# jacobkrantz/IVLN-CE

Hardware: AMD Instinct MI355X
Metric: env-steps/sec (batched MapCMA fwd+bwd) at 1/2/4/8 MI355X; t-nDTW parity (higher is better)
Workload: dtype f32

## Files before the change

### include/ivln_hip.h

```cpp
#ifndef IVLN_HIP_H
#define IVLN_HIP_H
#include <stdint.h>
#ifdef __cplusplus
extern "C" {
#endif

#define IVLN_OK 0
#define IVLN_E_INVALID -1
#define IVLN_E_HIP -2
#define IVLN_E_KEYSPACE -3
#define IVLN_E_CAPACITY -4
#define IVLN_E_UNSUPPORTED -5

const char* ivln_strerror(int code);
int ivln_version(void);

typedef struct ivln_mapper ivln_mapper;

int ivln_mapper_create(int B_max, int H, int W, double vfov_rad, double height_m, double width_m,
                       double res_m, int64_t world_capacity, int64_t table_cells, ivln_mapper** out);
int ivln_mapper_destroy(ivln_mapper* m);
int ivln_mapper_reset(ivln_mapper* m, void* stream);

int ivln_mapper_set_launch_width(ivln_mapper* m, int local_blocks, int world_blocks);

int ivln_mapper_frames(const float* pose, const double* orientation, int B, float* T, float* rot,
                       void* stream);

int ivln_mapper_step(ivln_mapper* m, const float* depth, const uint8_t* labels, const float* T,
                     const float* pose, const float* rot, const uint8_t* not_done, int B,
                     uint8_t* occ_out, uint8_t* sem_out, void* stream);

int ivln_mapper_step_posed(ivln_mapper* m, const float* depth, const uint8_t* labels, const float* pose,
                           const double* orientation, const uint8_t* not_done, int B, uint8_t* occ_out,
                           uint8_t* sem_out, float* T_out, float* rot_out, void* stream);

int ivln_mapper_step_begin(ivln_mapper* m, const float* depth, const float* pose, const double* orientation,
                           const uint8_t* not_done, int B, uint8_t* occ_out, float* T_out, float* rot_out, void* stream);
int ivln_mapper_step_finish(ivln_mapper* m, const float* depth, const uint8_t* labels, const float* T, const float* pose,
                            const float* rot, const uint8_t* not_done, int B, uint8_t* occ_out, uint8_t* sem_out, void* stream);

int ivln_mapper_known_begin(ivln_mapper* m, const uint8_t* not_done, int B, void* stream);
int ivln_mapper_load_known(ivln_mapper* m, int b, const float* xyz, const uint8_t* sem, int64_t n,
                           void* stream);
int ivln_mapper_known_raster(ivln_mapper* m, const float* pose, const float* rot, int B,
                             uint8_t* occ_out, uint8_t* sem_out, void* stream);

int ivln_mapper_status(ivln_mapper* m, int64_t* world_n, void* stream);
int ivln_mapper_world_export(ivln_mapper* m, float* xyz, uint32_t* meta, int64_t* rank,
                             int64_t max_n, int64_t* n_out, void* stream);


enum { IVLN_A_MK = 0,
       IVLN_A_KM = 1,
       IVLN_A_NCHW_P = 2    };
enum { IVLN_B_CONV = 0,
       IVLN_B_CONV1X1 = 1,
       IVLN_B_KN = 2,
       IVLN_B_NK = 3,
       IVLN_B_IM2COL_T = 4,
       IVLN_B_CONVT = 5,
       IVLN_B_CONV_K3 = 6,
       IVLN_B_CONV_K7 = 7,
       IVLN_B_CONV_K2 = 8   };
enum { IVLN_D_NCHW = 0,
       IVLN_D_DENSE = 1,
       IVLN_D_NCHW_UP2 = 2,
       IVLN_D_NCHW_UP2X4 = 3  };

typedef struct ivln_gemm_desc {
    const float* A;
    const float* B;
    float* D;
    int M, N, K;
    int amode, bmode, dmode;
    int64_t lda, ldb;
    int Cin, Hin, Win, Hout, Wout, stride, pad, dil;
    const int32_t* koff;
    const int32_t* kpos;
    int HoWo;
    int Ctot;
    int64_t in_img_stride;
    int64_t sDm, sDn;
    const float* scale;
    const float* shift;
    const float* residual;
    int relu, accumulate;
    int splits;
    float* ws;
    int64_t ws_floats;
    int defer_epilogue;
    int* splits_used;
    int tile_override;
    const float* A_packed;
    int no_xcd_remap;
    int grp_imgs;
    int64_t a_grp_stride, a_packed_grp_stride;
    int no_wide_epilogue;
    float* stat_partials;
    int* stat_tiles;
    const void* A_split;
    int64_t a_split_grp_stride;
    int split_ok;
    const int32_t* img_run_flags;
    const void* fuse_A_split;
    int64_t fuse_a_grp_stride;
    const float* fuse_scale;
    const float* fuse_shift;
    int fuse_M;
    int residual_after_relu;
    int real_taps;
} ivln_gemm_desc;

int ivln_gemm_f32(const ivln_gemm_desc* desc, void* stream);
int64_t ivln_conv_split_words(int M, int Cin, int KS);
int ivln_conv_split_weights_f32(const float* W, int M, int Cin, int KS, void* out, void* stream);
int64_t ivln_conv_stem_split_words(int M, int Cin);
int ivln_conv_stem_split_weights_f32(const float* W, int M, int Cin, void* out, void* stream);
int ivln_conv_split_counters(double* flops, long long* launches, int reset);
int ivln_conv_split_kinds(long long* out4, int reset);

int ivln_family_timing_begin(int max_launches);
int ivln_family_timing_end(double* total_ms, int* launches, int* dropped);
int ivln_family_timing_report(char* buf, int cap);
const char* ivln_family_kernel_names(void);
int64_t ivln_conv_packed_floats(int M, int Cin, int KS);
int ivln_conv_pack_weights_f32(const float* W, int M, int Cin, int KS, float* out, void* stream);

typedef struct ivln_gn_conv_desc {
    const float* x;
    int splits;
    int64_t slab_stride;
    const float* gamma;
    const float* beta;
    const float* x2;
    int splits2;
    int64_t slab_stride2;
    const float* gamma2;
    const float* beta2;
    const float* residual;
    int N, C, H, W, groups;
    float eps;
    int relu;
    int pool;
    float* act_out;
    const float* wa;
    int Cout_a, ka, stride_a, pad_a;
    float* ya;
    const float* wb;
    int Cout_b, stride_b;
    float* yb;
    const float* x0;
    int splits0;
    int64_t slab_stride0;
    int C0, groups0;
    const float* gamma0;
    const float* beta0;
    const float* w0;
} ivln_gn_conv_desc;
int ivln_gn_conv_f32(const ivln_gn_conv_desc* d, void* stream);

typedef struct ivln_depthnet_op {
    int kind;
    int Cin, Cout, ks, stride, pad;
    int Hin, Win;
    int wout_shift;
    int M;
    int WCT, WPT, P, KW;
    int kwg;
    int n_ctg, n_ptg;
    int ksteps;
    int cs, wp;
    int src_off, nslab, slab_stride;
    int st_off, st_parts;
    int gamma_off, beta_off;
    int src2_off, st2_off, st2_parts, gamma2_off, beta2_off;
    int res_off;
    int relu, pool, avg_in;
    int act_out_off;
    int dst_off, dst_slab_stride;
    int st_out_off, st_out_parts;
    int w_off;
    int barrier_before;
} ivln_depthnet_op;
int ivln_depth_net_f32(const ivln_depthnet_op* ops_dev, const ivln_depthnet_op* ops_host, int n_ops, const float* weights,
                       const float* params, const float* depth, int64_t depth_img_stride, float* arena, int64_t arena_stride,
                       float* out, int64_t out_img_stride, int N, float eps, void* sync_ws, void* stream);
int ivln_depth_net_status(const void* sync_ws, void* stream);
int ivln_depth_net_reset(void* sync_ws, void* stream);
int ivln_host_device_ptr(void* host, void** dev);

typedef struct ivln_nconv_desc {
    const float* x;
    const float* stats;
    int parts;
    const float* gamma;
    const float* beta;
    const float* x2;
    const float* stats2;
    int parts2;
    const float* gamma2;
    const float* beta2;
    const float* residual;
    int N, C, H, W, groups;
    float eps;
    int relu;
    float* act_out;
    const float* wa;
    int Cout_a, ka, groups_a;
    float* ya;
    float* stats_a;
    const float* wb;
    int Cout_b, groups_b;
    float* yb;
    float* stats_b;
    int rows_per_block;
    int stride_a, stride_b;
} ivln_nconv_desc;
int ivln_nconv_f32(const ivln_nconv_desc* d, void* stream);

int ivln_groupnorm_f32(const float* x, const float* gamma, const float* beta, const float* residual,
// ... 210 lines not shown
```

### ivln-ce_amd/csrc/conv_bf3.hip

```cpp
#include <stdlib.h>

#include <type_traits>

#include "gemm_common.h"
#include "residency.h"

namespace {

typedef __bf16 bf16x8 __attribute__((ext_vector_type(8)));
typedef int v4i __attribute__((ext_vector_type(4)));
typedef int v2i __attribute__((ext_vector_type(2)));

constexpr int PIXB = 112;
constexpr int CB = 16;

__host__ __device__ constexpr int bf3_taps_padded(int KS) { return KS == 7 ? 54 : (KS == 3 ? 9 : (KS == 2 ? 4 : 1)); }
__host__ __device__ constexpr int bf3_gx0(int KS) { return KS == 2 ? 0 : 4; }
__host__ __device__ constexpr int bf3_xoff(int KS) { return KS == 2 ? 0 : 4 - KS / 2; }
__host__ __device__ constexpr int bf3_stage_chunks(int KS) { return KS == 1 ? 4 : 1; }

__device__ __forceinline__ uint32_t bf16_rne_bits(float v, bool& fin) {
    const uint32_t u = __float_as_uint(v);
    fin = (u & 0x7F800000u) != 0x7F800000u;
    uint32_t hb = (u + 0x7FFFu + ((u >> 16) & 1u)) & 0xFFFF0000u;
// ... 720 lines not shown
                for (int pl = 0; pl < 3; ++pl) abuf[slot][pl] = load_a(s0 + r + DA, pl);
                if (r == (KK > 4 ? 1 : 0)) load_patch(min(c + 1, c1 - 1));
                __builtin_amdgcn_sched_barrier(0);
            }
        }
    }
#ifdef BF3_TIMING
    const unsigned long long ts2 = lane == 0 ? wall_clock64() : 0ull;
#endif
    __syncthreads();
    float* const red = reinterpret_cast<float*>(smem);
#pragma unroll
    for (int tn = 0; tn < TN; ++tn)
#pragma unroll
        for (int r = 0; r < 16; ++r)
            red[(wave * 32 + (r & 3) + 8 * (r >> 2) + 4 * half) * LDT + tn * 32 + l31] = acc[tn][r];
    __syncthreads();
    if constexpr (UP) {
        if (t < 16 * 16 * TN) {
            const int r = t / (16 * TN), j = t % (16 * TN);
            const int ml = 2 * r, nl = 2 * j;
            const int ph = nl / PTW, pw = nl % PTW;
            const int ho = ho0 + ph, wo = wo0 + pw;
            float4 v = make_float4(0.f, 0.f, 0.f, 0.f);
#pragma unroll
            for (int w = 0; w < NW; ++w) {
                const float2 u0 = *reinterpret_cast<const float2*>(red + (w * 32 + ml) * LDT + nl);
                const float2 u1 = *reinterpret_cast<const float2*>(red + (w * 32 + ml + 1) * LDT + nl);
                v.x += u0.x, v.y += u1.x, v.z += u0.y, v.w += u1.y;
            }
            if (m0 + ml < p.M && img0 < nimg && ho < p.Hout && wo < p.Wout) {
                const int co = (m0 + ml) >> 2, a = r & 1;
                const int64_t addr = (((int64_t)img0 * p.Ctot + co) * (2 * p.Hout) + 2 * ho + a) * (2 * p.Wout) + 2 * wo;
                if (p.scale) {
                    const float sc = p.scale[co], sh = p.shift[co];
                    v.x = fmaf(v.x, sc, sh), v.y = fmaf(v.y, sc, sh), v.z = fmaf(v.z, sc, sh), v.w = fmaf(v.w, sc, sh);
                } else if (p.shift) {
                    const float sh = p.shift[co];
                    v.x += sh, v.y += sh, v.z += sh, v.w += sh;
                }
                if (p.residual) {
                    const float4 rr = *reinterpret_cast<const float4*>(p.residual + addr);
                    v.x += rr.x, v.y += rr.y, v.z += rr.z, v.w += rr.w;
                }
                if (p.accumulate) {
                    const float4 rr = *reinterpret_cast<const float4*>(p.D + addr);
                    v.x += rr.x, v.y += rr.y, v.z += rr.z, v.w += rr.w;
                }
                if (p.relu) v.x = fmaxf(v.x, 0.f), v.y = fmaxf(v.y, 0.f), v.z = fmaxf(v.z, 0.f), v.w = fmaxf(v.w, 0.f);
                *reinterpret_cast<float4*>(p.D + addr) = v;
            }
        }
    } else if (t < 32 * 8 * TN) {
        const int ml = t / (8 * TN), c4 = t % (8 * TN);
        const int m = m0 + ml, nl = 4 * c4;
        const int ph = nl / PTW, pw = nl % PTW;
        const int ho = ho0 + ph, wo = wo0 + pw;
        float4 v = make_float4(0.f, 0.f, 0.f, 0.f);
#pragma unroll
        for (int w = 0; w < NW; ++w) {
            const float4 u = *reinterpret_cast<const float4*>(red + (w * 32 + ml) * LDT + nl);
            v.x += u.x, v.y += u.y, v.z += u.z, v.w += u.w;
        }
        if (m < p.M && img0 < nimg && ho < p.Hout && wo < p.Wout) {
            const int64_t addr = ((int64_t)img0 * p.Ctot + m) * p.HoWo + ho * p.Wout + wo;
            const int me = p.grp_imgs > 0 ? (img0 / p.grp_imgs) * p.M + m : m;
            if (p.scale) {
                const float sc = p.scale[me], sh = p.shift[me];
                v.x = fmaf(v.x, sc, sh), v.y = fmaf(v.y, sc, sh), v.z = fmaf(v.z, sc, sh), v.w = fmaf(v.w, sc, sh);
            } else if (p.shift) {
                const float sh = p.shift[me];
                v.x += sh, v.y += sh, v.z += sh, v.w += sh;
            }
            if (p.residual) {
                const float4 rr = *reinterpret_cast<const float4*>(p.residual + addr);
                v.x += rr.x, v.y += rr.y, v.z += rr.z, v.w += rr.w;
            }
            if (p.accumulate) {
                const float4 rr = *reinterpret_cast<const float4*>(p.D + addr);
                v.x += rr.x, v.y += rr.y, v.z += rr.z, v.w += rr.w;
            }
            if (p.relu) v.x = fmaxf(v.x, 0.f), v.y = fmaxf(v.y, 0.f), v.z = fmaxf(v.z, 0.f), v.w = fmaxf(v.w, 0.f);
            *reinterpret_cast<float4*>(p.D + addr) = v;
        }
    }
#ifdef BF3_TIMING
    if (lane == 0) {
        __builtin_amdgcn_s_waitcnt(0);
        const unsigned long long ts3 = wall_clock64();
        const int b = ((blockIdx.y * gridDim.x + blockIdx.x) * NW + wave) & 8191;
        g_bf3_stamp[b * 8 + 0] = ts1 - ts0;
        g_bf3_stamp[b * 8 + 1] = ts2 - ts1;
        g_bf3_stamp[b * 8 + 2] = ts3 - ts2;
        g_bf3_stamp[b * 8 + 3] = ts0;
        g_bf3_stamp[b * 8 + 4] = t_stage;
    }
#endif
}

template <int PTH, int PTW, int TN = 2, int KS = 3>
int launch_bf3_ks_tile(const ivln_gemm_desc& d, hipStream_t s, const unsigned char* a_split, int64_t grp_bytes, int nimg) {
    constexpr int NPIX = (PTH + KS - 1) * (PTW + KS - 1), WREG = (NPIX * PIXB + 15) & ~15, RED = 8 * 32 * (32 * TN + 4) * 4;
    constexpr size_t lds = (size_t)(8 * WREG > RED ? 8 * WREG : RED);
    static_assert(lds <= 160 * 1024, "patch regions do not fit");
    auto kern = k_conv_bf3_ks<PTH, PTW, TN, KS>;
    static bool attr_done = false;
    if (!attr_done) {
        if (hipFuncSetAttribute((const void*)kern, hipFuncAttributeMaxDynamicSharedMemorySize, (int)lds) != hipSuccess) return IVLN_E_HIP;
        attr_done = true;
    }
    const int tiles_w = d.Wout / PTW, tiles_h = d.Hout / PTH;
    dim3 grid(tiles_w * tiles_h * nimg, (d.M + 31) / 32, 1);
    IVLN_LAUNCH_FAMILY_NAMED("k_conv_bf3_ks", kern, grid, dim3(512), lds, s, d, a_split, (long long)grp_bytes, tiles_w, tiles_h, nimg);
    return IVLN_OK;
}

int bf3_ks_launch(ivln_gemm_desc& d, hipStream_t s, int nimg, int mode, int tn_pin = 0) {
    if (d.Cin % CB != 0 || d.Cin < 8 * CB || d.stat_partials || d.splits > 1) return IVLN_E_UNSUPPORTED;
    if (d.bmode == BMODE_CONV_K2) {
        if (d.grp_imgs > 0 || (d.Wout != 8 && d.Wout != 16 && d.Wout != 32) || d.Hout % (64 / d.Wout) != 0 || (d.in_img_stride & 3) ||
            (((uintptr_t)d.B) & 15) || (int64_t)nimg * d.in_img_stride * 4 >= (int64_t)1 << 31)
            return IVLN_E_UNSUPPORTED;
        const int64_t wgs2 = (int64_t)(d.N / 64) * ((d.M + 31) / 32);
        if (mode == 0 && (wgs2 > 2 * (int64_t)ivln_cu_count() || wgs2 < ivln_cu_count() / 4)) return IVLN_E_UNSUPPORTED;
        d.splits = 1;
        const unsigned char* a2 = (const unsigned char*)d.A_split;
        const int64_t gb2 = d.a_split_grp_stride * 4;
        if (d.Wout == 8) return launch_bf3_ks_tile<8, 8, 2, 2>(d, s, a2, gb2, nimg);
        if (d.Wout == 16) return launch_bf3_ks_tile<4, 16, 2, 2>(d, s, a2, gb2, nimg);
        return launch_bf3_ks_tile<2, 32, 2, 2>(d, s, a2, gb2, nimg);
    }
    if (d.Wout != 8 && d.Wout != 16 && d.Wout != 32) return IVLN_E_UNSUPPORTED;
    const int64_t wgs = (int64_t)(d.N / 64) * ((d.M + 31) / 32);
    constexpr int tn_env = 0;
    const bool small = tn_pin ? tn_pin == 1 : (tn_env ? tn_env == 1 : 2 * wgs <= ivln_cu_count());
    const int pth = (small ? 32 : 64) / d.Wout;
    if (d.Hout % pth != 0 || (d.in_img_stride & 3) || (((uintptr_t)d.B) & 15)) return IVLN_E_UNSUPPORTED;
    if ((int64_t)nimg * d.in_img_stride * 4 >= (int64_t)1 << 31) return IVLN_E_UNSUPPORTED;
    if (d.grp_imgs > 0 && nimg % d.grp_imgs != 0) return IVLN_E_UNSUPPORTED;
    if (mode == 0 && (wgs > 2 * (int64_t)ivln_cu_count() || wgs < ivln_cu_count() / 4)) return IVLN_E_UNSUPPORTED;
    const int64_t gb = d.a_split_grp_stride * 4;
    d.splits = 1;
    const unsigned char* a = (const unsigned char*)d.A_split;
    if (small) {
        if (d.Wout == 8) return launch_bf3_ks_tile<4, 8, 1>(d, s, a, gb, nimg);
        if (d.Wout == 16) return launch_bf3_ks_tile<2, 16, 1>(d, s, a, gb, nimg);
        return launch_bf3_ks_tile<1, 32, 1>(d, s, a, gb, nimg);
    }
    if (d.Wout == 8) return launch_bf3_ks_tile<8, 8>(d, s, a, gb, nimg);
    if (d.Wout == 16) return launch_bf3_ks_tile<4, 16>(d, s, a, gb, nimg);
    return launch_bf3_ks_tile<2, 32>(d, s, a, gb, nimg);
}

template <bool WT>
__global__ __launch_bounds__(WT ? 256 : 512, 2) void k_conv1x1_bf3_ks(const ivln_gemm_desc p, const unsigned char* a_split, long long a_grp_bytes) {
    constexpr int NW = WT ? 4 : 8, TN = 4, DA = 4, BN = 128;
    constexpr int LDT = BN + 4;
    constexpr unsigned OOB = 0x80000000u;
    extern __shared__ __attribute__((aligned(16))) unsigned char smem[];
    const int t = threadIdx.x, lane = t & 63;
    const int wave = __builtin_amdgcn_readfirstlane(t >> 6);
    const int half = lane >> 5, l31 = lane & 31;
    const BlockId bid = xcd_block_id(p.no_xcd_remap);
    const int n0 = WT ? (bid.y * NW + wave) * BN : bid.y * BN, m0 = bid.x * 32;
    const int nch = p.Cin / CB;
    const int HW = p.HoWo;
    const int cpw = WT ? nch : (nch + NW - 1) / NW;
    const int c0 = WT ? 0 : min(nch, wave * cpw), c1 = WT ? nch : min(nch, c0 + cpw);
    const int n_img0 = min(n0, p.N - 1) / HW;
    const int grp = p.grp_imgs > 0 ? n_img0 / p.grp_imgs : 0;

    const int nq = n0 + 4 * l31;
    const int qimg = nq / HW, qpp = nq - qimg * HW;
    const unsigned hw4 = (unsigned)HW * 4u;
    const unsigned xvo = nq < p.N ? (unsigned)(((int64_t)qimg * p.in_img_stride + qpp + (int64_t)(8 * half) * HW) * 4) : OOB;
    const __amdgpu_buffer_rsrc_t rB = bf3_rsrc(p.B);
    auto load_x = [&](int c, v4i (&xb)[8]) {
        const int so = c * CB * HW * 4;
#pragma unroll
        for (int j = 0; j < 8; ++j) xb[j] = __builtin_amdgcn_raw_buffer_load_b128(rB, (int)xvo, so + j * (int)hw4, 0);
    };
    const int mt = min(m0 / 32, (p.M + 31) / 32 - 1);
    const __amdgpu_buffer_rsrc_t rA = bf3_rsrc(a_split + (int64_t)grp * a_grp_bytes + (int64_t)mt * nch * (3 * 1024));
    const int c_last = max(c1 - 1, 0);
    auto load_a = [&](int c, v4i (&ab)[3]) {
#pragma unroll
        for (int pl = 0; pl < 3; ++pl) ab[pl] = __builtin_amdgcn_raw_buffer_load_b128(rA, (min(c, c_last) * 3 + pl) * 1024 + lane * 16, 0, 0);
    };
    f32x16 acc[TN];
#pragma unroll
    for (int tn = 0; tn < TN; ++tn)
#pragma unroll
        for (int i = 0; i < 16; ++i) acc[tn][i] = 0.f;

#ifdef BF3_TIMING
    const unsigned long long ts0 = lane == 0 ? wall_clock64() : 0ull;
    unsigned long long ts1 = ts0, tc_split = 0, tc_load = 0, tc_mfma = 0;
#endif
    if (c0 < c1 && (!WT || n0 < p.N)) {
        v4i xb[2][8], ab[DA][3];
#pragma unroll
        for (int d = 0; d < DA; ++d) load_a(c0 + d, ab[d]);
        load_x(c0, xb[0]);
        load_x(min(c0 + 1, c_last), xb[1]);
#ifdef BF3_TIMING
        __builtin_amdgcn_s_waitcnt(0);
        ts1 = lane == 0 ? wall_clock64() : 0ull;
#endif
        for (int cc = c0; cc < c1; cc += DA) {
#pragma unroll
            for (int k = 0; k < DA; ++k) {
                const int c = cc + k;
                v4i bq[TN][3];
                bf16x8 a[3];
#ifdef BF3_TIMING
                const unsigned long long tl0 = __builtin_readcyclecounter();
#endif
                if (c < c1) {
#pragma unroll
                    for (int e = 0; e < 4; ++e)
#pragma unroll
                        for (int i = 0; i < 4; ++i) {
                            uint32_t H, M, L;
#ifdef BF3_PROBE_NO_SPLIT
                            H = xb[k & 1][2 * i][e], M = xb[k & 1][2 * i + 1][e], L = H ^ M;
#else
                            split3_pair(__int_as_float(xb[k & 1][2 * i][e]), __int_as_float(xb[k & 1][2 * i + 1][e]), H, M, L);
#endif
                            bq[e][0][i] = (int)H, bq[e][1][i] = (int)M, bq[e][2][i] = (int)L;
                        }
#pragma unroll
                    for (int pl = 0; pl < 3; ++pl) a[pl] = __builtin_bit_cast(bf16x8, ab[k][pl]);
                }
                __builtin_amdgcn_sched_barrier(0);
#ifdef BF3_TIMING
                const unsigned long long tl1 = __builtin_readcyclecounter();
                __builtin_amdgcn_sched_barrier(0);
#endif
                load_x(min(c + 2, c_last), xb[k & 1]);
                load_a(c + DA, ab[k]);
                __builtin_amdgcn_sched_barrier(0);
#ifdef BF3_TIMING
                const unsigned long long tl2 = __builtin_readcyclecounter();
                __builtin_amdgcn_sched_barrier(0);
#endif
                if (c < c1) {
#define IVLN_BF3_PROD(PA, PB)                            \
    _Pragma("unroll") for (int tn = 0; tn < TN; ++tn)    \
        acc[tn] = __builtin_amdgcn_mfma_f32_32x32x16_bf16(a[PA], __builtin_bit_cast(bf16x8, bq[tn][PB]), acc[tn], 0, 0, 0)
#ifdef BF3_PROBE_NO_MFMA
                    IVLN_BF3_PROD(0, 0);
#else
                    IVLN_BF3_PROD(0, 2);
                    IVLN_BF3_PROD(1, 1);
                    IVLN_BF3_PROD(2, 0);
                    IVLN_BF3_PROD(0, 1);
                    IVLN_BF3_PROD(1, 0);
                    IVLN_BF3_PROD(0, 0);
#endif
#undef IVLN_BF3_PROD
                }
#ifdef BF3_TIMING
                __builtin_amdgcn_sched_barrier(0);
                const unsigned long long tl3 = __builtin_readcyclecounter();
                tc_split += tl1 - tl0, tc_load += tl2 - tl1, tc_mfma += tl3 - tl2;
#endif
            }
        }
    }
#ifdef BF3_TIMING
    const unsigned long long ts2 = lane == 0 ? wall_clock64() : 0ull;
#endif
    const bool up = p.dmode == DMODE_NCHW_UP2X4;
    if (WT && up) {
        const int n = n0 + 4 * l31;
        if (n < p.N) {
            const int img = n / HW, pp = n - img * HW;
            const int ho = pp / p.Wout, wo = pp - ho * p.Wout;
#pragma unroll
            for (int r = 0; r < 16; r += 2) {
                const int m = m0 + 4 * half + (r & 3) + 8 * (r >> 2);
                if (m >= p.M) continue;
                const int co = m >> 2, a = (m >> 1) & 1;
                const int64_t addr = (((int64_t)img * p.Ctot + co) * (2 * p.Hout) + 2 * ho + a) * (2 * p.Wout) + 2 * wo;
                float v[8];
#pragma unroll
                for (int e = 0; e < 4; ++e) v[2 * e] = acc[e][r], v[2 * e + 1] = acc[e][r + 1];
                const float sc = p.scale ? p.scale[co] : 1.f, sh = p.shift ? p.shift[co] : 0.f;
#pragma unroll
                for (int e = 0; e < 8; ++e) v[e] = p.scale ? fmaf(v[e], sc, sh) : v[e] + sh;
                if (p.residual) {
                    const float4 r0 = *reinterpret_cast<const float4*>(p.residual + addr), r1 = *reinterpret_cast<const float4*>(p.residual + addr + 4);
                    v[0] += r0.x, v[1] += r0.y, v[2] += r0.z, v[3] += r0.w, v[4] += r1.x, v[5] += r1.y, v[6] += r1.z, v[7] += r1.w;
                }
                if (p.relu) {
#pragma unroll
                    for (int e = 0; e < 8; ++e) v[e] = fmaxf(v[e], 0.f);
                }
                *reinterpret_cast<float4*>(p.D + addr) = make_float4(v[0], v[1], v[2], v[3]);
                *reinterpret_cast<float4*>(p.D + addr + 4) = make_float4(v[4], v[5], v[6], v[7]);
            }
        }
    } else
    if constexpr (WT) {
        const int n = n0 + 4 * l31;
        const int img = min(n, p.N - 1) / HW, pp = n - img * HW;
        const int mrem = n < p.N ? p.M - m0 - 4 * half : 0;
        const int me0 = (p.grp_imgs > 0 ? (img / p.grp_imgs) * p.M : 0) + m0 + 4 * half;
        const unsigned off0 = (unsigned)(((img * p.Ctot + m0 + 4 * half) * HW + pp) * 4);
        const __amdgpu_buffer_rsrc_t rR = bf3_rsrc(p.residual), rS = bf3_rsrc(p.scale), rH = bf3_rsrc(p.shift), rD = bf3_rsrc(p.D);
        const bool has_res = p.residual != nullptr, has_sc = p.scale != nullptr, has_sh = p.shift != nullptr;
        const float relu_lo = p.relu ? 0.f : -__builtin_huge_valf();
        const bool res_post = p.residual_after_relu != 0;
        v4i rres[16];
        float esc[16], esh[16];
#pragma unroll
        for (int r = 0; r < 16; ++r) {
            const int cs = (r & 3) + 8 * (r >> 2);
            const bool ok = cs < mrem;
            esc[r] = __int_as_float(__builtin_amdgcn_raw_buffer_load_b32(rS, ok && has_sc ? me0 * 4 : (int)OOB, cs * 4, 0));
            esh[r] = __int_as_float(__builtin_amdgcn_raw_buffer_load_b32(rH, ok && has_sh ? me0 * 4 : (int)OOB, cs * 4, 0));
            rres[r] = __builtin_amdgcn_raw_buffer_load_b128(rR, ok && has_res ? (int)off0 : (int)OOB, cs * HW * 4, 0);
        }
#pragma unroll
        for (int r = 0; r < 16; ++r) {
            const int cs = (r & 3) + 8 * (r >> 2);
            float4 v = make_float4(acc[0][r], acc[1][r], acc[2][r], acc[3][r]);
            const float sc = has_sc ? esc[r] : 1.f, sh = esh[r];
            v.x = fmaf(v.x, sc, sh), v.y = fmaf(v.y, sc, sh), v.z = fmaf(v.z, sc, sh), v.w = fmaf(v.w, sc, sh);
            const float r0 = __int_as_float(rres[r][0]), r1 = __int_as_float(rres[r][1]), r2 = __int_as_float(rres[r][2]), r3 = __int_as_float(rres[r][3]);
            v.x += res_post ? 0.f : r0, v.y += res_post ? 0.f : r1, v.z += res_post ? 0.f : r2, v.w += res_post ? 0.f : r3;
            const float lo = relu_lo;
            v.x = fmaxf(v.x, lo), v.y = fmaxf(v.y, lo), v.z = fmaxf(v.z, lo), v.w = fmaxf(v.w, lo);
            v.x += res_post ? r0 : 0.f, v.y += res_post ? r1 : 0.f, v.z += res_post ? r2 : 0.f, v.w += res_post ? r3 : 0.f;
            v4i o;
            o[0] = __float_as_int(v.x), o[1] = __float_as_int(v.y), o[2] = __float_as_int(v.z), o[3] = __float_as_int(v.w);
            __builtin_amdgcn_raw_buffer_store_b128(o, rD, cs < mrem ? (int)off0 : (int)OOB, cs * HW * 4, 0);
            BF3_STORE_GUARD();
        }
    } else if (up) {
        float* const red = reinterpret_cast<float*>(smem);
#pragma unroll
        for (int tn = 0; tn < TN; ++tn)
#pragma unroll
            for (int r = 0; r < 16; ++r)
                red[(wave * 32 + (r & 3) + 8 * (r >> 2) + 4 * half) * LDT + tn * 32 + l31] = acc[tn][r];
        __syncthreads();
#pragma unroll
        for (int it = 0; it < 2; ++it) {
            const int item = t + it * 512, r = item >> 6, j = item & 63;
            const int ml = 2 * r, nl = 2 * j, n = n0 + nl;
            const int e0 = nl & 3, q = nl >> 2;
            float4 v = make_float4(0.f, 0.f, 0.f, 0.f);
#pragma unroll
            for (int w = 0; w < NW; ++w) {
                const float* r0 = red + (w * 32 + ml) * LDT + q;
                const float* r1 = r0 + LDT;
                v.x += r0[e0 * 32], v.y += r1[e0 * 32], v.z += r0[(e0 + 1) * 32], v.w += r1[(e0 + 1) * 32];
            }
            if (m0 + ml < p.M && n < p.N) {
                const int img = n / HW, pp = n - img * HW;
                const int ho = pp / p.Wout, wo = pp - ho * p.Wout;
                const int co = (m0 + ml) >> 2, a = r & 1;
                const int64_t addr = (((int64_t)img * p.Ctot + co) * (2 * p.Hout) + 2 * ho + a) * (2 * p.Wout) + 2 * wo;
                if (p.scale) {
                    const float sc = p.scale[co], sh = p.shift[co];
                    v.x = fmaf(v.x, sc, sh), v.y = fmaf(v.y, sc, sh), v.z = fmaf(v.z, sc, sh), v.w = fmaf(v.w, sc, sh);
                } else if (p.shift) {
                    const float sh = p.shift[co];
                    v.x += sh, v.y += sh, v.z += sh, v.w += sh;
                }
                if (p.residual) {
                    const float4 rr = *reinterpret_cast<const float4*>(p.residual + addr);
                    v.x += rr.x, v.y += rr.y, v.z += rr.z, v.w += rr.w;
                }
                if (p.relu) v.x = fmaxf(v.x, 0.f), v.y = fmaxf(v.y, 0.f), v.z = fmaxf(v.z, 0.f), v.w = fmaxf(v.w, 0.f);
                *reinterpret_cast<float4*>(p.D + addr) = v;
            }
        }
    } else {
    constexpr int ITEMS = 2;
    v4i rres[ITEMS];
    float esc[ITEMS], esh[ITEMS];
    int eoff[ITEMS];
    const __amdgpu_buffer_rsrc_t rR = bf3_rsrc(p.residual), rS = bf3_rsrc(p.scale), rH = bf3_rsrc(p.shift);
    const bool has_res = p.residual != nullptr, has_sc = p.scale != nullptr, has_sh = p.shift != nullptr;
    auto request = [&](int it) {
        const int item = t + it * 512, ml = item >> 5, q = item & 31;
        const int m = m0 + ml, n = n0 + 4 * q;
        const bool ok = m < p.M && n < p.N;
        const int img = n / HW, pp = n - img * HW;
        const int off = (img * p.Ctot + m) * HW + pp;
        const int me = p.grp_imgs > 0 ? (img / p.grp_imgs) * p.M + m : m;
        eoff[it] = ok ? off : -1;
        esc[it] = __int_as_float(__builtin_amdgcn_raw_buffer_load_b32(rS, ok && has_sc ? me * 4 : (int)OOB, 0, 0));
        esh[it] = __int_as_float(__builtin_amdgcn_raw_buffer_load_b32(rH, ok && has_sh ? me * 4 : (int)OOB, 0, 0));
        rres[it] = __builtin_amdgcn_raw_buffer_load_b128(rR, ok && has_res ? off * 4 : (int)OOB, 0, 0);
    };
#pragma unroll
    for (int it = 0; it < ITEMS; ++it) request(it);
    float* const red = reinterpret_cast<float*>(smem);
#pragma unroll
    for (int tn = 0; tn < TN; ++tn)
#pragma unroll
        for (int r = 0; r < 16; ++r)
            red[(wave * 32 + (r & 3) + 8 * (r >> 2) + 4 * half) * LDT + tn * 32 + l31] = acc[tn][r];
    __syncthreads();
#pragma unroll
    for (int it = 0; it < ITEMS; ++it) {
        const int item = t + it * 512, ml = item >> 5, q = item & 31;
        float4 v = make_float4(0.f, 0.f, 0.f, 0.f);
#pragma unroll
        for (int w = 0; w < NW; ++w) {
            const float* rr = red + (w * 32 + ml) * LDT + q;
            v.x += rr[0], v.y += rr[32], v.z += rr[64], v.w += rr[96];
        }
        if (eoff[it] >= 0) {
            const int64_t addr = eoff[it];
            const float sc = esc[it], sh = esh[it];
            if (p.scale) v.x = fmaf(v.x, sc, sh), v.y = fmaf(v.y, sc, sh), v.z = fmaf(v.z, sc, sh), v.w = fmaf(v.w, sc, sh);
            else if (p.shift) v.x += sh, v.y += sh, v.z += sh, v.w += sh;
            const bool res_pre = p.residual && !p.residual_after_relu, res_post = p.residual && p.residual_after_relu;
            if (res_pre)
                v.x += __int_as_float(rres[it][0]), v.y += __int_as_float(rres[it][1]), v.z += __int_as_float(rres[it][2]),
                    v.w += __int_as_float(rres[it][3]);
            if (p.accumulate) {
                const float4 ra = *reinterpret_cast<const float4*>(p.D + addr);
                v.x += ra.x, v.y += ra.y, v.z += ra.z, v.w += ra.w;
            }
            if (p.relu) v.x = fmaxf(v.x, 0.f), v.y = fmaxf(v.y, 0.f), v.z = fmaxf(v.z, 0.f), v.w = fmaxf(v.w, 0.f);
            if (res_post)
                v.x += __int_as_float(rres[it][0]), v.y += __int_as_float(rres[it][1]), v.z += __int_as_float(rres[it][2]),
                    v.w += __int_as_float(rres[it][3]);
            *reinterpret_cast<float4*>(p.D + addr) = v;
        }
    }
    }
#ifdef BF3_TIMING
    if (lane == 0) {
        __builtin_amdgcn_s_waitcnt(0);
        const unsigned long long ts3 = wall_clock64();
        const int b = ((blockIdx.y * gridDim.x + blockIdx.x) * NW + wave) & 8191;
        g_bf3_stamp[b * 8 + 0] = ts1 - ts0;
        g_bf3_stamp[b * 8 + 1] = ts2 - ts1;
        g_bf3_stamp[b * 8 + 2] = ts3 - ts2;
        g_bf3_stamp[b * 8 + 3] = ts0;
        g_bf3_stamp[b * 8 + 4] = tc_split;
        g_bf3_stamp[b * 8 + 5] = tc_load;
        g_bf3_stamp[b * 8 + 6] = tc_mfma;
    }
#endif
}

int bf3_1x1_ks_launch(ivln_gemm_desc& d, hipStream_t s, int mode, int form_pin = -1) {
    if (d.stride != 1 || d.pad != 0 || d.Cin % CB != 0 || d.Cin < 4 * CB || d.stat_partials || d.splits > 1) return IVLN_E_UNSUPPORTED;
    if ((d.HoWo & 3) || (d.in_img_stride & 3) || ((((uintptr_t)d.B) | ((uintptr_t)d.D) | ((uintptr_t)d.residual)) & 15)) return IVLN_E_UNSUPPORTED;
    const int64_t nimg = d.N / d.HoWo;
    if (nimg * d.in_img_stride * 4 >= (int64_t)1 << 31 || nimg * d.Ctot * d.HoWo * 4 >= (int64_t)1 << 31) return IVLN_E_UNSUPPORTED;
    if (d.grp_imgs > 0 && ((int64_t)d.grp_imgs * d.HoWo) % 128 != 0) return IVLN_E_UNSUPPORTED;
    const int nch = d.Cin / CB;
    constexpr const char* form_env = nullptr;
    bool wt = nch <= 16;
    constexpr int maxwg0 = 2;
    if (nch == 32 && (int64_t)((d.N + 127) / 128) * ((d.M + 31) / 32) > maxwg0 * (int64_t)ivln_cu_count()) wt = true;
    if (form_env) wt = form_env[0] == 'w';
    if (form_pin >= 0) wt = form_pin == 1;
    if (wt && nch > 64) wt = false;
    if (wt && d.accumulate) return IVLN_E_UNSUPPORTED;
    const int64_t mtiles = (d.M + 31) / 32;
    const int64_t wgs = wt ? (int64_t)((d.N + 511) / 512) * mtiles : (int64_t)((d.N + 127) / 128) * mtiles;
    constexpr int maxwg_env = 2;
    if ((d.N + 127) / 128 > 65535) return IVLN_E_UNSUPPORTED;
    if (mode == 0) {
        if (!wt && (d.Cin < 32 * CB || wgs > maxwg_env * (int64_t)ivln_cu_count() || wgs < ivln_cu_count() / 2)) return IVLN_E_UNSUPPORTED;
        if (wt && wgs < ivln_cu_count()) return IVLN_E_UNSUPPORTED;
    }
    d.splits = 1;
    const unsigned char* a = (const unsigned char*)d.A_split;
    const long long gb = (long long)(d.a_split_grp_stride * 4);
    if (wt) {
        constexpr size_t lds = 0;
        dim3 grid((unsigned)mtiles, (unsigned)((d.N + 511) / 512), 1);
        IVLN_LAUNCH_FAMILY(k_conv1x1_bf3_ks<true>, grid, dim3(256), lds, s, d, a, gb);
    } else {
        constexpr size_t lds = (size_t)8 * 32 * (128 + 4) * 4;
        static bool attr_done = false;
        if (!attr_done) {
            if (hipFuncSetAttribute((const void*)k_conv1x1_bf3_ks<false>, hipFuncAttributeMaxDynamicSharedMemorySize, (int)lds) != hipSuccess) return IVLN_E_HIP;
            attr_done = true;
        }
        dim3 grid((unsigned)mtiles, (unsigned)((d.N + 127) / 128), 1);
        IVLN_LAUNCH_FAMILY(k_conv1x1_bf3_ks<false>, grid, dim3(512), lds, s, d, a, gb);
    }
    return IVLN_OK;
}

__global__ __launch_bounds__(256) void k_conv_bf3_pack(const float* __restrict__ W, int M, int Cin, int KS, uint16_t* __restrict__ out,
                                                       int64_t total) {
    const int64_t idx = (int64_t)blockIdx.x * 256 + threadIdx.x;
    if (idx >= total) return;
    const int KK = KS * KS, KKP = bf3_taps_padded(KS), nch = (Cin + CB - 1) / CB;
    const int e = (int)(idx & 7), lane = (int)((idx >> 3) & 63);
    int64_t q = idx >> 9;
    const int pl = (int)(q % 3);
    q /= 3;
    const int r = (int)(q % KKP);
    q /= KKP;
    const int c = (int)(q % nch);
    const int mt = (int)(q / nch);
    const int m = mt * 32 + (lane & 31), ci = c * CB + (lane >> 5) * 8 + e;
    const float v = (m < M && ci < Cin && r < KK) ? W[((int64_t)m * Cin + ci) * KK + r] : 0.f;
    uint32_t h, mm, l;
    split3(v, h, mm, l);
    out[idx] = (uint16_t)(pl == 0 ? h : (pl == 1 ? mm : l));
}

template <int KS, int TM, int WM, int WN, int PTH, int PTW, int IMGS, int DA, int ST = 1>
int launch_bf3(const ivln_gemm_desc& d, hipStream_t s, const unsigned char* a_split, int64_t grp_bytes, int nimg, int cps) {
    constexpr int NTB = 64 * WM * WN, BM = 32 * TM * WM, BN = 64 * WN;
    constexpr int PH = ST == 2 ? PTH + 1 : PTH + KS - 1, PWR = ST == 2 ? PTW + 1 : PTW + KS - 1;
    constexpr int NPIX = IMGS * (ST == 2 ? 4 : 1) * PH * PWR * bf3_stage_chunks(KS);
    constexpr size_t lds = (size_t)(NPIX * PIXB > 32 * (BN + 4) * 4 ? NPIX * PIXB : 32 * (BN + 4) * 4);
    if constexpr (lds > 160 * 1024) {
        return IVLN_E_UNSUPPORTED;
    } else {
    auto kern = k_conv_bf3<KS, TM, WM, WN, PTH, PTW, IMGS, DA, false, ST>;
    static bool attr_done = false;
    if (!attr_done) {
        if (hipFuncSetAttribute((const void*)kern, hipFuncAttributeMaxDynamicSharedMemorySize, (int)lds) != hipSuccess) return IVLN_E_HIP;
        attr_done = true;
    }
    const int tiles_w = (d.Wout + PTW - 1) / PTW, tiles_h = (d.Hout + PTH - 1) / PTH;
    const int groups = (nimg + IMGS - 1) / IMGS;
    dim3 grid(tiles_w * tiles_h * groups, (d.M + BM - 1) / BM, d.splits);
    IVLN_LAUNCH_FAMILY_NAMED("k_conv_bf3", kern, grid, dim3(NTB), lds, s, d, a_split, (long long)grp_bytes, tiles_w, tiles_h, nimg, cps);
    return IVLN_OK;
    }
}

template <int TM, int WM, int WN, int DA>
int launch_bf3_fused(const ivln_gemm_desc& d, hipStream_t s, const unsigned char* a_split, int64_t grp_bytes, int nimg) {
    constexpr int KS = 3, PTW = 32, NTB = 64 * WM * WN, BM = 32 * TM * WM, BN = 64 * WN, PTH = BN / PTW;
    static_assert(NTB == 256, "four waves");
    constexpr int NPIX = (PTH + 2) * (PTW + 2);
    constexpr size_t ybytes = (size_t)BM * (BN + 4) * 4, lds = (size_t)NPIX * PIXB > ybytes ? (size_t)NPIX * PIXB : ybytes;
    auto kern = k_conv_bf3<KS, TM, WM, WN, PTH, PTW, 1, DA, true>;
    static bool attr_done = false;
    if (!attr_done) {
        if (hipFuncSetAttribute((const void*)kern, hipFuncAttributeMaxDynamicSharedMemorySize, (int)lds) != hipSuccess) return IVLN_E_HIP;
        attr_done = true;
    }
    const int tiles_w = d.Wout / PTW, tiles_h = d.Hout / PTH;
    dim3 grid(tiles_w * tiles_h * nimg, 1, 1);
    const int nch = d.Cin / CB;
    IVLN_LAUNCH_FAMILY_NAMED("k_conv_bf3", kern, grid, dim3(NTB), lds, s, d, a_split, (long long)grp_bytes, tiles_w, tiles_h, nimg, nch);
    return IVLN_OK;
}

struct Bf3Px { int pth, ptw, imgs; };
inline Bf3Px bf3_px(int BN, int Wout) {
    const int ptw = Wout > 16 ? 32 : (Wout > 8 ? 16 : 8);
    const int pth = ptw == 32 ? BN / 32 : (ptw == 16 ? (BN >= 256 ? 16 : 8) : 8);
    return {pth, ptw, BN / (ptw * pth)};
}

template <int KS, int TM, int WM, int WN, int DA, int ST = 1>
int launch_bf3_px(const ivln_gemm_desc& d, hipStream_t s, const unsigned char* a, int64_t gb, int nimg, int cps) {
    constexpr int BN = 64 * WN;
    if constexpr (ST == 2) {
        static_assert(KS == 3 && (BN == 128 || BN == 256), "stride-2 tiles");
        if constexpr (BN == 256) {
            if (d.Wout > 16) return launch_bf3<KS, TM, WM, WN, 8, 32, 1, DA, 2>(d, s, a, gb, nimg, cps);
            if (d.Wout > 8) return launch_bf3<KS, TM, WM, WN, 16, 16, 1, DA, 2>(d, s, a, gb, nimg, cps);
            return launch_bf3<KS, TM, WM, WN, 8, 8, 4, DA, 2>(d, s, a, gb, nimg, cps);
        } else {
            if (d.Wout > 16) return launch_bf3<KS, TM, WM, WN, 4, 32, 1, DA, 2>(d, s, a, gb, nimg, cps);
            if (d.Wout > 8) return launch_bf3<KS, TM, WM, WN, 8, 16, 1, DA, 2>(d, s, a, gb, nimg, cps);
            return launch_bf3<KS, TM, WM, WN, 8, 8, 2, DA, 2>(d, s, a, gb, nimg, cps);
        }
    } else
    if constexpr (BN == 512 && KS == 1) {
        return IVLN_E_UNSUPPORTED;
    } else if constexpr (BN == 512) {
        if (d.Wout > 16) return launch_bf3<KS, TM, WM, WN, 16, 32, 1, DA>(d, s, a, gb, nimg, cps);
        if (d.Wout > 8) return launch_bf3<KS, TM, WM, WN, 16, 16, 2, DA>(d, s, a, gb, nimg, cps);
        if constexpr (KS == 3) return launch_bf3<KS, TM, WM, WN, 8, 8, 8, DA>(d, s, a, gb, nimg, cps);
        return IVLN_E_UNSUPPORTED;
    } else if constexpr (BN == 256) {
        if (d.Wout > 16) return launch_bf3<KS, TM, WM, WN, 8, 32, 1, DA>(d, s, a, gb, nimg, cps);
        if (d.Wout > 8) return launch_bf3<KS, TM, WM, WN, 16, 16, 1, DA>(d, s, a, gb, nimg, cps);
        return launch_bf3<KS, TM, WM, WN, 8, 8, 4, DA>(d, s, a, gb, nimg, cps);
    } else {
        if (d.Wout > 16) return launch_bf3<KS, TM, WM, WN, 4, 32, 1, DA>(d, s, a, gb, nimg, cps);
        if (d.Wout > 8) return launch_bf3<KS, TM, WM, WN, 8, 16, 1, DA>(d, s, a, gb, nimg, cps);
        return launch_bf3<KS, TM, WM, WN, 8, 8, 2, DA>(d, s, a, gb, nimg, cps);
    }
}

constexpr int kBf3Cfgs = 7;
constexpr int kBf3BM[kBf3Cfgs] = {32, 64, 64, 128, 64, 128, 32};
constexpr int kBf3BN[kBf3Cfgs] = {512, 512, 256, 256, 128, 128, 256};

template <int KS>
int launch_bf3_ks(const ivln_gemm_desc& d, hipStream_t s, const unsigned char* a, int64_t gb, int nimg, int cfg, int cps) {
    constexpr int DA2 = KS == 1 || KS == 2 ? 2 : 3, DA1 = KS == 1 || KS == 2 ? 4 : (KS == 7 ? 2 : 3);
    if constexpr (KS == 2) {
        switch (cfg) {
            case 2: return launch_bf3_px<KS, 1, 2, 4, DA1>(d, s, a, gb, nimg, cps);
            case 3: return launch_bf3_px<KS, 2, 2, 4, DA2>(d, s, a, gb, nimg, cps);
            case 4: return launch_bf3_px<KS, 1, 2, 2, DA1>(d, s, a, gb, nimg, cps);
            case 5: return launch_bf3_px<KS, 2, 2, 2, DA2>(d, s, a, gb, nimg, cps);
            default: return IVLN_E_UNSUPPORTED;
        }
    }
    switch (cfg) {
        case 0: return launch_bf3_px<KS, 1, 1, 8, DA1>(d, s, a, gb, nimg, cps);
        case 1: return launch_bf3_px<KS, 2, 1, 8, DA2>(d, s, a, gb, nimg, cps);
        case 2: return launch_bf3_px<KS, 1, 2, 4, DA1>(d, s, a, gb, nimg, cps);
        case 3: return launch_bf3_px<KS, 2, 2, 4, DA2>(d, s, a, gb, nimg, cps);
        case 4: return launch_bf3_px<KS, 1, 2, 2, DA1>(d, s, a, gb, nimg, cps);
        case 5: return launch_bf3_px<KS, 2, 2, 2, DA2>(d, s, a, gb, nimg, cps);
        default: return launch_bf3_px<KS, 1, 1, 4, DA1>(d, s, a, gb, nimg, cps);
    }
}


int launch_bf3_s2(const ivln_gemm_desc& d, hipStream_t s, const unsigned char* a, int64_t gb, int nimg, int cfg, int cps) {
    switch (cfg) {
        case 2: return launch_bf3_px<3, 1, 2, 4, 3, 2>(d, s, a, gb, nimg, cps);
        case 3: return launch_bf3_px<3, 2, 2, 4, 3, 2>(d, s, a, gb, nimg, cps);
        case 4: return launch_bf3_px<3, 1, 2, 2, 3, 2>(d, s, a, gb, nimg, cps);
        case 5: return launch_bf3_px<3, 2, 2, 2, 3, 2>(d, s, a, gb, nimg, cps);
        case 6: return launch_bf3_px<3, 1, 1, 4, 3, 2>(d, s, a, gb, nimg, cps);
        default: return IVLN_E_UNSUPPORTED;
    }
}


template <int TM, int WM, int WN, int W, bool XE = false>
__global__ __launch_bounds__(64 * WM * WN, XE ? 3 : 1) void k_wgrad_bf3(const ivln_gemm_desc p, int nimg, int strips_total, int strips_per_split) {
    constexpr int NTB = 64 * WM * WN, TN = 2, KS = 7, KK = 49;
    constexpr int NPX = XE ? 1 : 3;
    constexpr int BM = 32 * TM * WM, BN = 32 * TN * WN;
    constexpr int IMS = W == 8 ? 2 : 1, ROWS = 128 / (W * IMS);
    constexpr int PR = ROWS + KS - 1, PRT = IMS * PR, PWP = W + KS - 1;
// ... 322 lines not shown
        for (int s = 0; s < S; ++s) {
            if (s + 2 < S) load_a(s + 2, ab[(s + 2) % 3]), load_x(s + 2, xb[(s + 2) % 3]);
            uint32_t Hh[7], Mm[7], Ll[7];
#pragma unroll
            for (int u = 0; u < 7; ++u) {
                const int i0 = 2 * u + 1, i1 = 2 * u + 2;
                split3_pair(__int_as_float(xb[s % 3][i0 >> 2][i0 & 3]), __int_as_float(xb[s % 3][i1 >> 2][i1 & 3]), Hh[u], Mm[u], Ll[u]);
            }
            v4i bq[TN][3];
#pragma unroll
            for (int e = 0; e < TN; ++e)
#pragma unroll
                for (int i = 0; i < 4; ++i) bq[e][0][i] = (int)Hh[e + i], bq[e][1][i] = (int)Mm[e + i], bq[e][2][i] = (int)Ll[e + i];
            bf16x8 a[3];
#pragma unroll
            for (int pl = 0; pl < 3; ++pl) a[pl] = __builtin_bit_cast(bf16x8, ab[s % 3][pl]);
#define IVLN_BF3_PROD(PA, PB)                            \
    _Pragma("unroll") for (int tn = 0; tn < TN; ++tn)    \
        acc[tn] = __builtin_amdgcn_mfma_f32_32x32x16_bf16(a[PA], __builtin_bit_cast(bf16x8, bq[tn][PB]), acc[tn], 0, 0, 0)
            IVLN_BF3_PROD(0, 2);
            IVLN_BF3_PROD(1, 1);
            IVLN_BF3_PROD(2, 0);
            IVLN_BF3_PROD(0, 1);
            IVLN_BF3_PROD(1, 0);
            IVLN_BF3_PROD(0, 0);
#undef IVLN_BF3_PROD
        }
    }
    const int pp = ho * p.Wout + 128 * seg + 4 * l31;
    const int mrem = p.M - m0 - 4 * half;
    const int me0 = m0 + 4 * half;
    const unsigned off0 = (unsigned)(((img * p.Ctot + m0 + 4 * half) * HW + pp) * 4);
    const __amdgpu_buffer_rsrc_t rR = bf3_rsrc(p.residual), rS = bf3_rsrc(p.scale), rH = bf3_rsrc(p.shift), rD = bf3_rsrc(p.D);
    const bool has_res = p.residual != nullptr, has_sc = p.scale != nullptr, has_sh = p.shift != nullptr;
    const float relu_lo = p.relu ? 0.f : -__builtin_huge_valf();
    const bool res_post = p.residual_after_relu != 0;
    v4i rres[16];
    float esc[16], esh[16];
#pragma unroll
    for (int r = 0; r < 16; ++r) {
        const int cs = (r & 3) + 8 * (r >> 2);
        const bool ok = cs < mrem;
        esc[r] = __int_as_float(__builtin_amdgcn_raw_buffer_load_b32(rS, ok && has_sc ? me0 * 4 : (int)OOB, cs * 4, 0));
        esh[r] = __int_as_float(__builtin_amdgcn_raw_buffer_load_b32(rH, ok && has_sh ? me0 * 4 : (int)OOB, cs * 4, 0));
        rres[r] = __builtin_amdgcn_raw_buffer_load_b128(rR, ok && has_res ? (int)off0 : (int)OOB, cs * HW * 4, 0);
    }
#pragma unroll
    for (int r = 0; r < 16; ++r) {
        const int cs = (r & 3) + 8 * (r >> 2);
        float4 v = make_float4(acc[0][r], acc[1][r], acc[2][r], acc[3][r]);
        const float sc = has_sc ? esc[r] : 1.f, sh = esh[r];
        v.x = fmaf(v.x, sc, sh), v.y = fmaf(v.y, sc, sh), v.z = fmaf(v.z, sc, sh), v.w = fmaf(v.w, sc, sh);
        const float r0 = __int_as_float(rres[r][0]), r1 = __int_as_float(rres[r][1]), r2 = __int_as_float(rres[r][2]), r3 = __int_as_float(rres[r][3]);
        v.x += res_post ? 0.f : r0, v.y += res_post ? 0.f : r1, v.z += res_post ? 0.f : r2, v.w += res_post ? 0.f : r3;
        const float lo = relu_lo;
        v.x = fmaxf(v.x, lo), v.y = fmaxf(v.y, lo), v.z = fmaxf(v.z, lo), v.w = fmaxf(v.w, lo);
        v.x += res_post ? r0 : 0.f, v.y += res_post ? r1 : 0.f, v.z += res_post ? r2 : 0.f, v.w += res_post ? r3 : 0.f;
        v4i o;
        o[0] = __float_as_int(v.x), o[1] = __float_as_int(v.y), o[2] = __float_as_int(v.z), o[3] = __float_as_int(v.w);
        __builtin_amdgcn_raw_buffer_store_b128(o, rD, cs < mrem ? (int)off0 : (int)OOB, cs * HW * 4, 0);
        BF3_STORE_GUARD();
    }
}

__global__ __launch_bounds__(256) void k_conv7s2_pack(const float* __restrict__ W, int M, int Cin, uint16_t* __restrict__ out, int64_t total) {
    const int64_t idx = (int64_t)blockIdx.x * 256 + threadIdx.x;
    if (idx >= total) return;
    const int S = (Cin * 7 + 1) / 2;
    const int j = (int)(idx & 7), lane = (int)((idx >> 3) & 63);
    int64_t q = idx >> 9;
    const int pl = (int)(q % 3);
    q /= 3;
    const int st = (int)(q % S);
    const int mt = (int)(q / S);
    const int m = mt * 32 + (lane & 31), row = 2 * st + (lane >> 5);
    const float v = (m < M && row < Cin * 7 && j < 7) ? W[((int64_t)m * Cin * 7 + row) * 7 + j] : 0.f;
    uint32_t h, mm, l;
    split3(v, h, mm, l);
    out[idx] = (uint16_t)(pl == 0 ? h : (pl == 1 ? mm : l));
}

}

extern "C" int64_t ivln_conv_stem_split_words(int M, int Cin) {
    if (M <= 0 || (Cin != 1 && Cin != 3)) return 0;
    return (int64_t)((M + 31) / 32) * ((Cin * 7 + 1) / 2) * (3 * 1024 / 4);
}

extern "C" int ivln_conv_stem_split_weights_f32(const float* W, int M, int Cin, void* out, void* stream) {
    const int64_t words = ivln_conv_stem_split_words(M, Cin);
    if (!W || !out || words <= 0) return IVLN_E_INVALID;
    const int64_t total = words * 2;
    hipLaunchKernelGGL(k_conv7s2_pack, dim3((unsigned)((total + 255) / 256)), dim3(256), 0, (hipStream_t)stream, W, M, Cin, (uint16_t*)out, total);
    return hipGetLastError() == hipSuccess ? IVLN_OK : IVLN_E_HIP;
}

namespace {
int bf3_stem_launch(ivln_gemm_desc& d, hipStream_t s) {
    if ((d.Cin != 1 && d.Cin != 3) || d.pad != 3 || d.dil != 1 || d.Hin != 2 * d.Hout || d.Win != 2 * d.Wout || d.Wout % 128 != 0 ||
        d.K != d.Cin * 49 || d.HoWo != d.Hout * d.Wout || d.N % d.HoWo != 0 || d.dmode != DMODE_NCHW || d.amode != AMODE_MK)
        return IVLN_E_UNSUPPORTED;
    if (d.grp_imgs > 0 || d.accumulate || d.defer_epilogue || d.splits > 1 || d.stat_partials || d.img_run_flags || d.fuse_A_split)
        return IVLN_E_UNSUPPORTED;
    if ((d.in_img_stride & 3) || ((((uintptr_t)d.B) | ((uintptr_t)d.D) | ((uintptr_t)d.residual)) & 15)) return IVLN_E_UNSUPPORTED;
    const int64_t nimg = d.N / d.HoWo;
    if (nimg * d.in_img_stride * 4 >= (int64_t)1 << 31 || nimg * d.Ctot * d.HoWo * 4 >= (int64_t)1 << 31) return IVLN_E_UNSUPPORTED;
    const int segs = d.Wout / 128;
    const int64_t items = nimg * d.Hout * segs * ((d.M + 31) / 32);
    if (items >= (int64_t)1 << 30) return IVLN_E_UNSUPPORTED;
    d.splits = 1;
    const dim3 grid((unsigned)((items + 3) / 4));
    const unsigned char* a = (const unsigned char*)d.A_split;
    if (d.Cin == 3) IVLN_LAUNCH_FAMILY(k_conv7s2_bf3<3>, grid, dim3(256), 0, s, d, a, segs, (int)items);
    else IVLN_LAUNCH_FAMILY(k_conv7s2_bf3<1>, grid, dim3(256), 0, s, d, a, segs, (int)items);
    return IVLN_OK;
}
}

static double g_bf3_flops = 0.0;
static long long g_bf3_launches = 0;
static long long g_bf3_kind[4] = {0, 0, 0, 0};
extern "C" int ivln_conv_split_counters(double* flops, long long* launches, int reset) {
    if (flops) *flops = g_bf3_flops;
    if (launches) *launches = g_bf3_launches;
    if (reset) g_bf3_flops = 0.0, g_bf3_launches = 0;
    return IVLN_OK;
}
extern "C" int ivln_conv_split_kinds(long long* out4, int reset) {
    if (out4) for (int i = 0; i < 4; ++i) out4[i] = g_bf3_kind[i];
    if (reset) for (int i = 0; i < 4; ++i) g_bf3_kind[i] = 0;
    return IVLN_OK;
}

#ifdef BF3_TIMING
extern "C" int ivln_conv_bf3_stamps(unsigned long long* host, int n) {
    if (hipMemcpyFromSymbol(host, HIP_SYMBOL(g_bf3_stamp), sizeof(unsigned long long) * n) != hipSuccess) return -1;
    void* dp = nullptr;
    if (hipGetSymbolAddress(&dp, HIP_SYMBOL(g_bf3_stamp)) != hipSuccess) return -1;
    return hipMemset(dp, 0, sizeof(g_bf3_stamp)) == hipSuccess ? 0 : -1;
}
#endif

int ivln_conv_bf3_launch(ivln_gemm_desc& d, hipStream_t s, bool force) {
    constexpr bool disabled = false;
    if (!d.A_split || (disabled && !force)) return IVLN_E_UNSUPPORTED;
    const int KS = d.bmode == BMODE_CONV1X1 ? 1 : conv_ks(d.bmode);
    if ((KS != 1 && KS != 2 && KS != 3 && KS != 7) || d.amode != AMODE_MK || d.dil != 1) return IVLN_E_UNSUPPORTED;
    if (KS == 7 && d.stride == 2) {
        const int rc = bf3_stem_launch(d, s);
        if (rc == IVLN_OK) g_bf3_flops += 2.0 * d.M * (double)d.N * d.K, ++g_bf3_launches, ++g_bf3_kind[0];
        if (rc == IVLN_OK && d.stat_tiles) *d.stat_tiles = 0;
        return rc;
    }
    const bool up1 = KS == 1 && d.dmode == DMODE_NCHW_UP2X4;
    if (!up1 && d.dmode != (KS == 2 ? DMODE_NCHW_UP2X4 : DMODE_NCHW)) return IVLN_E_UNSUPPORTED;
    if (up1) {
        static const bool convt_off1 = getenv("IVLN_BF3_CONVT") && getenv("IVLN_BF3_CONVT")[0] == '0';
        if ((convt_off1 && !force) || (d.M & 3) || d.Ctot * 4 != d.M || d.grp_imgs > 0 || d.accumulate || d.residual_after_relu || d.defer_epilogue ||
            d.splits > 1 || d.stat_partials || d.img_run_flags || d.fuse_A_split || (d.Wout & 3) || d.stride != 1 || d.pad != 0 || d.Hout != d.Hin ||
            d.Wout != d.Win || d.K != d.Cin || d.HoWo != d.Hout * d.Wout || d.N % d.HoWo != 0)
            return IVLN_E_UNSUPPORTED;
        const int ovu = d.tile_override;
        const int rc = bf3_1x1_ks_launch(d, s, (force || ovu == 11 || ovu == 12 || ovu == 13) ? 1 : 0, ovu == 12 ? 0 : (ovu == 13 ? 1 : -1));
        if (rc == IVLN_OK) g_bf3_flops += 2.0 * d.M * (double)d.N * d.K, ++g_bf3_launches, ++g_bf3_kind[d.Cin / CB <= 16 ? 3 : 2];
        return rc;
    }
    const double flops_of = 2.0 * d.M * (double)d.N * d.K * (KS == 2 && d.real_taps > 0 ? d.real_taps / 16.0 : 1.0);
    if (KS == 2) {
        if (d.stride != 1 || d.pad != 0 || d.Hout != d.Hin || d.Wout != d.Win || (d.M & 3) || d.grp_imgs > 0 || d.stat_partials || d.defer_epilogue ||
            d.splits > 1 || d.fuse_A_split || d.residual_after_relu || d.img_run_flags || d.K != d.Cin * 4 || d.HoWo != d.Hout * d.Wout ||
            d.N % d.HoWo != 0 || (d.Wout & 3) || d.Wout < 8 || (((uintptr_t)d.D | (uintptr_t)d.residual) & 15) || d.Ctot * 4 != d.M)
            return IVLN_E_UNSUPPORTED;
        const int nimg2 = d.N / d.HoWo;
        if ((int64_t)nimg2 * d.in_img_stride >= (int64_t)1 << 31) return IVLN_E_UNSUPPORTED;
        static const bool convt_off = getenv("IVLN_BF3_CONVT") && getenv("IVLN_BF3_CONVT")[0] == '0';
        if (convt_off && !force) return IVLN_E_UNSUPPORTED;
        const int ov2 = d.tile_override;
        if (ov2 < 20) {
            const int rc = bf3_ks_launch(d, s, nimg2, (ov2 == 10 || ov2 == 15) ? 1 : 0);
            if (rc != IVLN_E_UNSUPPORTED || ov2 == 10 || ov2 == 15) {
                if (rc == IVLN_OK) g_bf3_flops += flops_of, ++g_bf3_launches, ++g_bf3_kind[1];
                return rc;
            }
        }
        const int CUS2 = ivln_cu_count();
        auto blocks2 = [&](int cfg) {
            const Bf3Px t = bf3_px(kBf3BN[cfg], d.Wout);
            return (int64_t)((d.Wout + t.ptw - 1) / t.ptw) * ((d.Hout + t.pth - 1) / t.pth) * ((nimg2 + t.imgs - 1) / t.imgs) *
                   ((d.M + kBf3BM[cfg] - 1) / kBf3BM[cfg]);
        };
        int cfg2 = blocks2(3) >= CUS2 ? 3 : (blocks2(2) >= CUS2 ? 2 : (blocks2(5) >= CUS2 ? 5 : 4));
        if (ov2 >= 20 && ov2 < 20 + kBf3Cfgs) cfg2 = ov2 - 20;
        if (!force && blocks2(cfg2) < CUS2 / 2) return IVLN_E_UNSUPPORTED;
        d.splits = 1;
        const int rc = launch_bf3_ks<2>(d, s, (const unsigned char*)d.A_split, d.a_split_grp_stride * 4, nimg2, cfg2, (d.Cin + CB - 1) / CB);
        if (rc == IVLN_OK) g_bf3_flops += flops_of, ++g_bf3_launches, ++g_bf3_kind[0];
        return rc;
    }
    static const int ks1_env = getenv("IVLN_BF3_1X1_KS") ? atoi(getenv("IVLN_BF3_1X1_KS")) : -1;
    const int ov = d.tile_override;
    const bool post = d.residual_after_relu != 0;
    const bool ins1 = ov == 11 || ov == 12 || ov == 13 || post, ins3 = ov == 10 || ov == 14 || ov == 15;
    if (KS == 1 && ov < 20 && (ks1_env != 0 || ins1) && d.splits <= 1 && !d.defer_epilogue && d.HoWo == d.Hout * d.Wout &&
        d.K == d.Cin && d.N % d.HoWo == 0 && d.Hout == d.Hin && d.Wout == d.Win) {
        const int rc = bf3_1x1_ks_launch(d, s, (ks1_env == 1 || ins1) ? 1 : 0, ov == 12 ? 0 : (ov == 13 ? 1 : -1));
        if (rc != IVLN_E_UNSUPPORTED || ins1) {
            if (rc == IVLN_OK) g_bf3_flops += 2.0 * d.M * (double)d.N * d.K, ++g_bf3_launches, ++g_bf3_kind[ov == 13 ? 3 : (ov == 12 ? 2 : (d.Cin / CB <= 16 ? 3 : 2))];
            if (rc == IVLN_OK && d.stat_tiles) *d.stat_tiles = 0;
            return rc;
        }
    }
    if (ins1 || (ins3 && KS != 3)) return IVLN_E_UNSUPPORTED;
    if (KS == 1) {
        if ((d.stride != 1 && d.stride != 2) || d.pad != 0 || d.Hout != (d.Hin - 1) / d.stride + 1 || d.Wout != (d.Win - 1) / d.stride + 1 || d.M < 64)
            return IVLN_E_UNSUPPORTED;
    } else if (KS == 3 && d.stride == 2) {
        static const bool s2_off = getenv("IVLN_BF3_S2") && getenv("IVLN_BF3_S2")[0] == '0';
        if ((s2_off && !force) || d.pad != 1 || d.Hin != 2 * d.Hout || d.Win != 2 * d.Wout || d.Cin % CB != 0 || d.fuse_A_split || d.stat_partials ||
            d.img_run_flags)
            return IVLN_E_UNSUPPORTED;
    } else if (d.stride != 1 || d.pad != KS / 2 || d.Hout != d.Hin || d.Wout != d.Win) {
        return IVLN_E_UNSUPPORTED;
    }
    const bool s2 = KS == 3 && d.stride == 2;
    if (d.K != d.Cin * KS * KS || d.HoWo != d.Hout * d.Wout || d.N % d.HoWo != 0) return IVLN_E_UNSUPPORTED;
    if (d.defer_epilogue || d.splits > 1 || (d.Wout & 3) || d.Wout < 8 || (((uintptr_t)d.D | (uintptr_t)d.residual | (uintptr_t)d.ws) & 15))
        return IVLN_E_UNSUPPORTED;
    const int nimg = d.N / d.HoWo;
    if ((int64_t)nimg * d.in_img_stride >= (int64_t)1 << 31) return IVLN_E_UNSUPPORTED;
    if (d.fuse_A_split) {
        static const bool fuse_off = getenv("IVLN_BF3_FUSE") && getenv("IVLN_BF3_FUSE")[0] == '0';
        if (fuse_off || KS != 3 || (d.M != 64 && d.M != 128) || d.Cin % CB != 0 || d.Wout % 32 != 0 || d.Hout % 4 != 0 || d.fuse_M <= 0 ||
            d.fuse_M % 32 != 0 || d.stat_partials || d.accumulate || !d.relu || d.img_run_flags)
            return IVLN_E_UNSUPPORTED;
        if ((int64_t)nimg * d.Ctot * d.HoWo * 4 >= (int64_t)1 << 31 || (d.grp_imgs > 0 && nimg % d.grp_imgs != 0)) return IVLN_E_UNSUPPORTED;
        d.splits = 1;
        const unsigned char* a = (const unsigned char*)d.A_split;
        const int64_t gb = d.a_split_grp_stride * 4;
        constexpr int px_env = 0;
        const int64_t wg128 = (int64_t)nimg * (d.Wout / 32) * (d.Hout / 4);
        const bool px64 = d.M == 128 && d.Hout % 2 == 0 && (px_env ? px_env == 64 : wg128 < ivln_cu_count());
        const int rc = d.M == 64 ? launch_bf3_fused<1, 2, 2, 3>(d, s, a, gb, nimg)
                       : (px64 ? launch_bf3_fused<1, 4, 1, 3>(d, s, a, gb, nimg) : launch_bf3_fused<2, 2, 2, 3>(d, s, a, gb, nimg));
        if (rc == IVLN_OK) g_bf3_flops += 2.0 * d.M * (double)d.N * d.K + 2.0 * d.fuse_M * (double)d.N * d.M, ++g_bf3_launches, ++g_bf3_kind[0];
        if (rc == IVLN_OK && d.stat_tiles) *d.stat_tiles = 0;
        return rc;
    }
    static const int ks_env = getenv("IVLN_BF3_KS") ? atoi(getenv("IVLN_BF3_KS")) : -1;
    if (KS == 3 && !s2 && ov < 20 && (ks_env != 0 || ins3) && d.splits <= 1) {
        const int rc = bf3_ks_launch(d, s, nimg, (ks_env == 1 || ins3) ? 1 : 0, ov == 14 ? 1 : (ov == 15 ? 2 : 0));
        if (rc != IVLN_E_UNSUPPORTED || ins3) {
            if (rc == IVLN_OK) g_bf3_flops += 2.0 * d.M * (double)d.N * d.K, ++g_bf3_launches, ++g_bf3_kind[1];
            if (rc == IVLN_OK && d.stat_tiles) *d.stat_tiles = 0;
            return rc;
        }
    }
    const int nch = ((d.Cin + CB - 1) / CB + bf3_stage_chunks(KS) - 1) / bf3_stage_chunks(KS);
    auto tiles_of = [&](int cfg) {
        const Bf3Px t = bf3_px(kBf3BN[cfg], d.Wout);
        return (int64_t)((d.Wout + t.ptw - 1) / t.ptw) * ((d.Hout + t.pth - 1) / t.pth) * ((nimg + t.imgs - 1) / t.imgs);
    };
    auto blocks_of = [&](int cfg) { return tiles_of(cfg) * ((d.M + kBf3BM[cfg] - 1) / kBf3BM[cfg]); };
    const int CUS = ivln_cu_count();
    auto fills = [&](int64_t nb, int slots) {
        const int64_t round = (int64_t)CUS * slots, rounds = (nb + round - 1) / round;
        return nb * 4 >= rounds * round * 3;
    };
    constexpr int cfg_env = -1;
    constexpr int split_env = 0;
    int cfg = -1, splits = 1;
    const bool big_ok = !(KS == 7 && d.Wout <= 8) && !s2;
    constexpr bool nosplit4 = true;
    constexpr int cfg32_env = -1;
    if (d.M <= 32) cfg = cfg32_env >= 0 ? cfg32_env : 6;
    else if (d.M <= 64)
        cfg = (big_ok && KS != 1 && fills(blocks_of(1), 1)) ? 1
              : (fills(blocks_of(2), 1) ? 2 : ((force || (nosplit4 && blocks_of(4) >= CUS)) ? 4 : -1));
    else cfg = fills(blocks_of(3), 1) ? 3 : (fills(blocks_of(2), 1) ? 2 : (((int64_t)d.M * d.N >= (1 << 21) && blocks_of(5) >= CUS) ? 5 : 4));
    if (cfg < 0) return IVLN_E_UNSUPPORTED;
    if (cfg_env >= 0 && cfg_env < kBf3Cfgs && !(cfg_env == 0 && d.M > 32)) cfg = cfg_env;
    if (d.tile_override >= 20 && d.tile_override < 20 + kBf3Cfgs) cfg = d.tile_override - 20;
    if ((cfg == 0 && !big_ok) || (KS == 1 && (cfg <= 1 || cfg == 6))) return IVLN_E_UNSUPPORTED;
    const int64_t nb = blocks_of(cfg);
    if (!force && (double)d.N < 0.15 * (double)tiles_of(cfg) * kBf3BN[cfg]) return IVLN_E_UNSUPPORTED;
    if (cfg >= 4) {
        const int slots = cfg == 4 ? 3 : 2;
        const bool may_split = d.splits == 0 && d.ws && nch >= 2 && !d.stat_partials;
        if (may_split && nb < (int64_t)CUS * slots && !(cfg == 4 && nosplit4 && nb >= CUS)) {
            const int64_t want = (int64_t)CUS * slots;
            splits = (int)((want + nb - 1) / nb);
            if (splits > nch) splits = nch;
            if (splits > 16) splits = 16;
            const int64_t cap = d.ws_floats / ((int64_t)d.M * d.N);
            if (splits > cap) splits = (int)cap;
            if (splits < 1) splits = 1;
        }
        if (split_env > 0 && may_split) {
            splits = split_env > nch ? nch : split_env;
            const int64_t cap = d.ws_floats / ((int64_t)d.M * d.N);
            if (splits > cap) splits = (int)cap;
            if (splits < 1) splits = 1;
        }
        if (!force && nb * splits < CUS * 3 / 4) return IVLN_E_UNSUPPORTED;
    } else if (!force && !fills(nb, cfg == 6 ? 2 : 1)) {
        return IVLN_E_UNSUPPORTED;
    }
    const int cps = (nch + splits - 1) / splits;
    splits = (nch + cps - 1) / cps;
    const Bf3Px t = bf3_px(kBf3BN[cfg], d.Wout);
    if (d.grp_imgs > 0 && (d.grp_imgs % t.imgs != 0 || nimg % d.grp_imgs != 0)) return IVLN_E_UNSUPPORTED;
    d.splits = splits;
    if (splits > 1) d.stat_partials = nullptr;
    const int64_t tiles = tiles_of(cfg);
    const int BN = kBf3BN[cfg];
    const int64_t gb = d.a_split_grp_stride * 4;
    const int rc = KS == 7   ? launch_bf3_ks<7>(d, s, (const unsigned char*)d.A_split, gb, nimg, cfg, cps)
                   : s2      ? launch_bf3_s2(d, s, (const unsigned char*)d.A_split, gb, nimg, cfg, cps)
                   : KS == 3 ? launch_bf3_ks<3>(d, s, (const unsigned char*)d.A_split, gb, nimg, cfg, cps)
                             : launch_bf3_ks<1>(d, s, (const unsigned char*)d.A_split, gb, nimg, cfg, cps);
    if (rc == IVLN_OK) g_bf3_flops += 2.0 * d.M * (double)d.N * d.K, ++g_bf3_launches, ++g_bf3_kind[0];
    if (rc == IVLN_OK && d.stat_tiles) *d.stat_tiles = d.stat_partials ? (int)(tiles * (BN / 128)) : 0;
    return rc;
}

int ivln_wgrad_bf3_launch(ivln_gemm_desc& d, hipStream_t s, bool force) {
    constexpr bool disabled = false;
    if ((!d.split_ok && !force) || (disabled && !force)) return IVLN_E_UNSUPPORTED;
    if (d.amode != AMODE_NCHW_P || d.bmode != BMODE_IM2COL_T || d.dmode != DMODE_DENSE || d.stride != 1 || d.dil != 1 || d.Cin <= 0 ||
        d.N != d.Cin * 49 || d.defer_epilogue || d.pad != 3)
        return IVLN_E_UNSUPPORTED;
    if (d.HoWo != d.Hout * d.Wout || d.K % d.HoWo != 0 || d.Hout != d.Hin || d.Wout != d.Win) return IVLN_E_UNSUPPORTED;
    if (d.Wout != 64 && d.Wout != 32 && d.Wout != 16 && d.Wout != 8) return IVLN_E_UNSUPPORTED;
    const int ims = d.Wout == 8 ? 2 : 1, rows = 128 / (d.Wout * ims);
    if (d.Hout % rows != 0 || (d.Wout == 8 && d.Hout != 8) || (((uintptr_t)d.A) & 7)) return IVLN_E_UNSUPPORTED;
    const int nimg = d.K / d.HoWo;
    if ((int64_t)nimg * d.in_img_stride >= (int64_t)1 << 31 || (int64_t)nimg * d.M * d.HoWo >= (int64_t)1 << 31) return IVLN_E_UNSUPPORTED;
    const int strips = ((nimg + ims - 1) / ims) * (d.Hout / rows);
    constexpr int l1_env = 0;
    const bool six = d.M <= 32 && (l1_env ? l1_env == 6 : (d.N + 383) / 384 * 384 < (d.N + 511) / 512 * 512);
    const bool xe = d.split_ok == 2 && d.M <= 32 && d.Wout == 64;
    const int BM = d.M <= 32 ? 32 : (d.M <= 64 ? 64 : 128), BN = xe ? 256 : (d.M <= 32 ? (six ? 384 : 512) : (d.M <= 64 ? 512 : 256));
    const int64_t blocks = (int64_t)((d.N + BN - 1) / BN) * ((d.M + BM - 1) / BM);
    if (!d.ws || d.ws_floats < (int64_t)d.M * d.N) return IVLN_E_UNSUPPORTED;
    int splits = 1;
    if (d.splits == 0) {
        if (d.ws) {
            constexpr int want_env = 0;
            const int64_t want = want_env > 0 ? want_env : (xe ? 3 : 1) * (int64_t)ivln_cu_count();
            splits = (int)(want / blocks);
            if (splits < 1) splits = 1;
            if (splits > strips) splits = strips;
            const int64_t cap = d.ws_floats / ((int64_t)d.M * d.N);
            if (splits > cap) splits = (int)cap;
            if (splits < 1) splits = 1;
        }
    } else {
        splits = d.splits > strips ? strips : d.splits;
        if (splits > 1 && (!d.ws || d.ws_floats < (int64_t)splits * d.M * d.N)) return IVLN_E_INVALID;
    }
    if (!force && blocks * splits < ivln_cu_count() / 2) return IVLN_E_UNSUPPORTED;
    const int sps = (strips + splits - 1) / splits;
    splits = (strips + sps - 1) / sps;
    d.splits = splits;
    int rc;
    if (xe) rc = launch_wgrad_bf3<1, 1, 4, 64, true>(d, s, nimg, strips, sps);
// ... 8 lines not shown
```

### ivln-ce_amd/csrc/gemm_common.h

```cpp
#pragma once
#include <hip/hip_runtime.h>
#include <stdint.h>
#include "../../include/ivln_hip.h"
#include "family_timing.h"

namespace {

typedef float f32x16 __attribute__((ext_vector_type(16)));

enum { AMODE_MK = 0, AMODE_KM = 1, AMODE_NCHW_P = 2 };
enum { BMODE_CONV = 0, BMODE_CONV1X1 = 1, BMODE_KN = 2, BMODE_NK = 3, BMODE_IM2COL_T = 4, BMODE_CONVT = 5,
       BMODE_CONV_K3 = 6, BMODE_CONV_K7 = 7,
       BMODE_CONV_K2 = 8 };
__host__ __device__ constexpr int conv_ks(int bmode) {
    return bmode == BMODE_CONV_K7 ? 7 : (bmode == BMODE_CONV_K3 ? 3 : (bmode == BMODE_CONV_K2 ? 2 : 0));
}
__host__ __device__ constexpr int conv_direct_ci(int KS) { return KS == 7 ? 2 : (KS == 2 ? 16 : 8); }
enum { DMODE_NCHW = 0, DMODE_DENSE = 1, DMODE_NCHW_UP2 = 2, DMODE_NCHW_UP2X4 = 3 };

__device__ __forceinline__ bool ivln_tile_skipped(const ivln_gemm_desc& p, int n0, int BN) {
    if (!p.img_run_flags) return false;
    const int last = min(p.N, n0 + BN) - 1;
    if (last < n0) return true;
    for (int i = n0 / p.HoWo; i <= last / p.HoWo; ++i)
        if (p.img_run_flags[i]) return false;
    return true;
}

constexpr int BK = 16;

struct BlockId {
    int x, y, z;
};
__device__ __forceinline__ BlockId xcd_block_id(int disabled) {
    BlockId b{(int)blockIdx.x, (int)blockIdx.y, (int)blockIdx.z};
    const int gx = gridDim.x, gy = gridDim.y;
    const int nwg = gx * gy * (int)gridDim.z;
    if (disabled || nwg < 16) return b;
    const int orig = (b.z * gy + b.y) * gx + b.x;
    const int xcd = orig & 7, q = nwg >> 3, r = nwg & 7;
    const int id = (xcd < r ? xcd * (q + 1) : r * (q + 1) + (xcd - r) * q) + (orig >> 3);
    const int t = id / gx;
    b.x = id - t * gx;
    b.z = t / gy;
    b.y = t - b.z * gy;
    return b;
}

__device__ __forceinline__ int tile_group(const ivln_gemm_desc& p, int n0) {
    return p.grp_imgs > 0 ? (n0 / p.HoWo) / p.grp_imgs : 0;
}

__device__ __forceinline__ void epilogue_store(const ivln_gemm_desc& p, int m, int n, float v) {
    int64_t addr;
    int me = m;
    if (p.dmode == DMODE_NCHW) {
        int img = n / p.HoWo;
        int pp = n - img * p.HoWo;
        addr = ((int64_t)img * p.Ctot + m) * p.HoWo + pp;
        if (p.grp_imgs > 0) me = (img / p.grp_imgs) * p.M + m;
    } else if (p.dmode == DMODE_NCHW_UP2) {
        int img = n / p.HoWo;
        int pp = n - img * p.HoWo;
        int ho = pp / p.Wout, wo = pp - ho * p.Wout;
        addr = (((int64_t)img * p.Ctot + m) * (2 * p.Hout) + 2 * ho + (int)p.sDm) * (2 * p.Wout) + 2 * wo + (int)p.sDn;
    } else if (p.dmode == DMODE_NCHW_UP2X4) {
        const int cls = m & 3;
        me = m >> 2;
        int img = n / p.HoWo;
        int pp = n - img * p.HoWo;
        int ho = pp / p.Wout, wo = pp - ho * p.Wout;
        addr = (((int64_t)img * p.Ctot + me) * (2 * p.Hout) + 2 * ho + (cls >> 1)) * (2 * p.Wout) + 2 * wo + (cls & 1);
    } else {
        addr = (int64_t)m * p.sDm + (int64_t)n * p.sDn;
    }
    if (p.scale) v = fmaf(v, p.scale[me], p.shift[me]);
    else if (p.shift) v += p.shift[me];
    if (p.residual) v += p.residual[addr];
    if (p.accumulate) v += p.D[addr];
    if (p.relu) v = fmaxf(v, 0.f);
    p.D[addr] = v;
}

__device__ __forceinline__ void epilogue_tile(const ivln_gemm_desc& p, int m_base, int n, int half, const f32x16& acc,
                                              int split_z) {
    const bool to_ws = p.splits > 1 || p.defer_epilogue;
    const bool vec4 = !to_ws && p.dmode == DMODE_DENSE && p.sDm == 1 && (p.sDn & 3) == 0 && (p.M & 3) == 0 &&
                      (((uintptr_t)p.D | (uintptr_t)p.residual) & 15) == 0;
    if (n >= p.N) return;
#pragma unroll
    for (int q = 0; q < 4; ++q) {
        const int m = m_base + 8 * q + 4 * half;
        if (vec4) {
            if (m >= p.M) continue;
            const int64_t addr = (int64_t)m + (int64_t)n * p.sDn;
            float v[4];
#pragma unroll
            for (int i = 0; i < 4; ++i) {
                v[i] = acc[4 * q + i];
                if (p.scale) v[i] = fmaf(v[i], p.scale[m + i], p.shift[m + i]);
                else if (p.shift) v[i] += p.shift[m + i];
            }
            if (p.residual) {
                const float4 r = *reinterpret_cast<const float4*>(p.residual + addr);
                v[0] += r.x, v[1] += r.y, v[2] += r.z, v[3] += r.w;
            }
            if (p.accumulate) {
                const float4 r = *reinterpret_cast<const float4*>(p.D + addr);
                v[0] += r.x, v[1] += r.y, v[2] += r.z, v[3] += r.w;
            }
            if (p.relu) {
#pragma unroll
                for (int i = 0; i < 4; ++i) v[i] = fmaxf(v[i], 0.f);
            }
            *reinterpret_cast<float4*>(p.D + addr) = make_float4(v[0], v[1], v[2], v[3]);
        } else {
#pragma unroll
            for (int i = 0; i < 4; ++i) {
                if (m + i < p.M) {
                    if (to_ws) p.ws[((int64_t)split_z * p.M + m + i) * p.N + n] = acc[4 * q + i];
                    else epilogue_store(p, m + i, n, acc[4 * q + i]);
                }
            }
        }
    }
}

template <int BM, int BN, int LDC, typename Pix>
__device__ __forceinline__ void up2x4_wide_store(const ivln_gemm_desc& p, const float* T, int m0, Pix pix) {
    constexpr int PAIRS = BN / 2;
    for (int f = threadIdx.x; f < (BM / 2) * PAIRS; f += 256) {
        const int j = f % PAIRS, r = f / PAIRS;
        const int ml = 2 * r;
        if (m0 + ml >= p.M) continue;
        int img, ho, wo;
        if (!pix(2 * j, img, ho, wo)) continue;
        const int co = (m0 + ml) >> 2, a = r & 1;
        const int64_t addr = (((int64_t)img * p.Ctot + co) * (2 * p.Hout) + 2 * ho + a) * (2 * p.Wout) + 2 * wo;
        const float2 t0 = *reinterpret_cast<const float2*>(T + ml * LDC + 2 * j);
        const float2 t1 = *reinterpret_cast<const float2*>(T + (ml + 1) * LDC + 2 * j);
        float4 v = make_float4(t0.x, t1.x, t0.y, t1.y);
        if (p.scale) {
            const float sc = p.scale[co], sh = p.shift[co];
            v.x = fmaf(v.x, sc, sh), v.y = fmaf(v.y, sc, sh), v.z = fmaf(v.z, sc, sh), v.w = fmaf(v.w, sc, sh);
        } else if (p.shift) {
            const float sh = p.shift[co];
            v.x += sh, v.y += sh, v.z += sh, v.w += sh;
        }
        if (p.residual) {
            const float4 rr = *reinterpret_cast<const float4*>(p.residual + addr);
            v.x += rr.x, v.y += rr.y, v.z += rr.z, v.w += rr.w;
        }
        if (p.accumulate) {
            const float4 rr = *reinterpret_cast<const float4*>(p.D + addr);
            v.x += rr.x, v.y += rr.y, v.z += rr.z, v.w += rr.w;
        }
        if (p.relu) v.x = fmaxf(v.x, 0.f), v.y = fmaxf(v.y, 0.f), v.z = fmaxf(v.z, 0.f), v.w = fmaxf(v.w, 0.f);
        *reinterpret_cast<float4*>(p.D + addr) = v;
    }
}
template <int BM, int BN, int LDC, typename Pix>
__device__ __forceinline__ void nchw_wide_store(const ivln_gemm_desc& p, const float* T, int m0, Pix pix,
                                                float* stats = nullptr) {
    static_assert(BN == 128 && (BM * (BN / 4)) % 256 == 0, "a row of the tile = the 32 lanes of a half-wave");
    for (int idx = threadIdx.x; idx < BM * (BN / 4); idx += 256) {
        const int ml = idx / (BN / 4), c4 = idx - ml * (BN / 4);
        const int m = m0 + ml;
        int img = 0, pp = 0;
        const bool ok = m < p.M && pix(4 * c4, img, pp);
        float4 v = make_float4(0.f, 0.f, 0.f, 0.f);
        if (ok) {
// ... 54 lines not shown
```

### ivln-ce_amd/csrc/gemm_conv.hip

```cpp
#include <stdlib.h>

#include <vector>
#include <string>
#include <string.h>
#include <stdio.h>

#include "gemm_common.h"

namespace {

template <int WM, int WN, int TM, int TN, int AMODE, int BMODE>
__global__ __launch_bounds__(256) void k_gemm(const ivln_gemm_desc p) {
    constexpr int BM = 32 * WM * TM, BN = 32 * WN * TN;
    constexpr int LDA_S = BM + 1, LDB_S = BN + 1;
    constexpr int EA = BM * BK / 256, EB = BN * BK / 256;
    __shared__ float smem[BK * LDA_S + BK * LDB_S];
    float* As = smem;
    float* Bs = smem + BK * LDA_S;

    const int t = threadIdx.x;
    const int lane = t & 63, wave = t >> 6;
    const int wm = wave / WN, wn = wave % WN;
    const BlockId bid = xcd_block_id(p.no_xcd_remap);
    const int m0 = bid.y * BM, n0 = bid.x * BN;
// ... 313 lines not shown
    if (p.relu) v.x = fmaxf(v.x, 0.f), v.y = fmaxf(v.y, 0.f), v.z = fmaxf(v.z, 0.f), v.w = fmaxf(v.w, 0.f);
    *reinterpret_cast<float4*>(p.D + q * 4) = v;
}

void launch_splitk_epilogue(const ivln_gemm_desc& d, hipStream_t s) {
    if (d.dmode == DMODE_DENSE && d.sDn == 1 && d.sDm == d.N && (((int64_t)d.M * d.N) & 3) == 0 && !d.scale && !d.shift &&
        !d.no_wide_epilogue && (((uintptr_t)d.D | (uintptr_t)d.residual | (uintptr_t)d.ws) & 15) == 0) {
        const int64_t total4 = (int64_t)d.M * d.N / 4;
        hipLaunchKernelGGL(k_splitk_epilogue_flat4, dim3((unsigned)((total4 + 63) / 64)), dim3(256), 0, s, d);
        return;
    }
    const bool lay = (d.dmode == DMODE_NCHW && (d.HoWo & 3) == 0) || (d.dmode == DMODE_DENSE && d.sDn == 1 && (d.sDm & 3) == 0);
    const bool vec4 = lay && (d.N & 3) == 0 && !d.no_wide_epilogue &&
                      (((uintptr_t)d.D | (uintptr_t)d.residual | (uintptr_t)d.ws) & 15) == 0;
    if (vec4) {
        const int64_t total = (int64_t)d.M * (d.N >> 2);
        hipLaunchKernelGGL(k_splitk_epilogue4, dim3((unsigned)((total + 255) / 256)), dim3(256), 0, s, d);
    } else {
        const int64_t total = (int64_t)d.M * d.N;
        hipLaunchKernelGGL(k_splitk_epilogue, dim3((unsigned)((total + 255) / 256)), dim3(256), 0, s, d);
    }
}

template <int WM, int WN, int TM, int TN>
int launch_tile(const ivln_gemm_desc& d, hipStream_t s) {
    constexpr int BM = 32 * WM * TM, BN = 32 * WN * TN;
    dim3 grid((d.N + BN - 1) / BN, (d.M + BM - 1) / BM, d.splits);
    dim3 block(256);
#define IVLN_CASE(AM, BMD)                                                              \
    if (d.amode == AM && d.bmode == BMD) {                                              \
        IVLN_LAUNCH_FAMILY((k_gemm<WM, WN, TM, TN, AM, BMD>), grid, block, 0, s, d);            \
        return IVLN_OK;                                                                 \
    }
    IVLN_CASE(AMODE_MK, BMODE_CONV)
    IVLN_CASE(AMODE_MK, BMODE_CONV1X1)
    IVLN_CASE(AMODE_MK, BMODE_CONV_K3)
    IVLN_CASE(AMODE_MK, BMODE_CONV_K7)
    IVLN_CASE(AMODE_MK, BMODE_CONV_K2)
    IVLN_CASE(AMODE_MK, BMODE_CONVT)
    IVLN_CASE(AMODE_MK, BMODE_NK)
    IVLN_CASE(AMODE_MK, BMODE_KN)
    IVLN_CASE(AMODE_KM, BMODE_NK)
    IVLN_CASE(AMODE_KM, BMODE_KN)
    IVLN_CASE(AMODE_NCHW_P, BMODE_IM2COL_T)
#undef IVLN_CASE
    return IVLN_E_UNSUPPORTED;
}

}

namespace {
const char* const kFamilyKernels[] = {"k_gemm",     "k_gemm_vec",    "k_conv_direct",    "k_wgrad_direct", "k_conv1x1_stream", "k_conv_bf3",
                                      "k_conv_bf3_ks", "k_conv1x1_bf3_ks", "k_conv7s2_bf3", "k_wgrad_bf3",    "k_gn_conv",        "k_nconv",
                                      "k_depth_net"};
constexpr int kFamilyCount = (int)(sizeof(kFamilyKernels) / sizeof(kFamilyKernels[0]));
std::vector<hipEvent_t> g_timing_events;
std::vector<int> g_timing_kernel;
int g_timing_used = -1;
int g_timing_dropped = 0;
double g_report_ms[kFamilyCount + 1];
int g_report_n[kFamilyCount + 1];
bool g_report_valid = false;

int family_index(const char* site) {
    while (*site == '(' || *site == ' ') ++site;
    size_t n = 0;
    while (site[n] && site[n] != '<' && site[n] != ')' && site[n] != ' ') ++n;
    for (int i = 0; i < kFamilyCount; ++i)
        if (strlen(kFamilyKernels[i]) == n && !strncmp(kFamilyKernels[i], site, n)) return i;
    return kFamilyCount;
}
}

bool ivln_family_timing_next(hipEvent_t* start, hipEvent_t* stop, const char* kernel) {
    if (g_timing_used < 0) return false;
    if ((size_t)g_timing_used + 2 > g_timing_events.size()) {
        ++g_timing_dropped;
        return false;
    }
    *start = g_timing_events[g_timing_used];
    *stop = g_timing_events[g_timing_used + 1];
    g_timing_kernel[g_timing_used / 2] = family_index(kernel);
    g_timing_used += 2;
    return true;
}

extern "C" const char* ivln_family_kernel_names(void) {
    static std::string names;
    if (names.empty())
        for (int i = 0; i < kFamilyCount; ++i) names += std::string(i ? "," : "") + kFamilyKernels[i];
    return names.c_str();
}

extern "C" int ivln_family_timing_begin(int max_launches) {
    if (max_launches <= 0 || g_timing_used >= 0) return IVLN_E_INVALID;
    while (g_timing_events.size() < (size_t)max_launches * 2) {
        hipEvent_t e;
        if (hipEventCreate(&e) != hipSuccess) return IVLN_E_HIP;
        g_timing_events.push_back(e);
    }
    g_timing_kernel.assign(g_timing_events.size() / 2, kFamilyCount);
    g_timing_used = 0;
    g_timing_dropped = 0;
    g_report_valid = false;
    return IVLN_OK;
}

extern "C" int ivln_family_timing_end(double* total_ms, int* launches, int* dropped) {
    if (g_timing_used < 0 || !total_ms || !launches) return IVLN_E_INVALID;
    const int used = g_timing_used;
    g_timing_used = -1;
    double sum = 0.0;
    for (int k = 0; k <= kFamilyCount; ++k) g_report_ms[k] = 0.0, g_report_n[k] = 0;
    for (int i = 0; i < used; i += 2) {
        if (hipEventSynchronize(g_timing_events[i + 1]) != hipSuccess) return IVLN_E_HIP;
        float ms = 0.f;
        if (hipEventElapsedTime(&ms, g_timing_events[i], g_timing_events[i + 1]) != hipSuccess) return IVLN_E_HIP;
        sum += ms;
        g_report_ms[g_timing_kernel[i / 2]] += ms;
        g_report_n[g_timing_kernel[i / 2]] += 1;
    }
    g_report_valid = true;
    *total_ms = sum;
    *launches = used / 2;
    if (dropped) *dropped = g_timing_dropped;
    return IVLN_OK;
}

extern "C" int ivln_family_timing_report(char* buf, int cap) {
    if (!g_report_valid) return IVLN_E_INVALID;
    std::string out;
    char line[128];
    for (int k = 0; k <= kFamilyCount; ++k) {
        if (!g_report_n[k]) continue;
        snprintf(line, sizeof line, "%s %d %.6f\n", k < kFamilyCount ? kFamilyKernels[k] : "?", g_report_n[k], g_report_ms[k]);
        out += line;
    }
    const int need = (int)out.size() + 1;
    if (!buf || cap < need) return need;
    memcpy(buf, out.c_str(), (size_t)need);
    return 0;
}

extern "C" int ivln_gemm_f32(const ivln_gemm_desc* desc, void* stream) {
    if (!desc || !desc->A || !desc->B || !desc->D || desc->M <= 0 || desc->N <= 0 || desc->K <= 0)
        return IVLN_E_INVALID;
    ivln_gemm_desc d = *desc;
    hipStream_t s = (hipStream_t)stream;
    static const bool no_xcd_env = getenv("IVLN_NO_XCD_REMAP") != nullptr;
    if (no_xcd_env) d.no_xcd_remap = 1;
    if (d.HoWo <= 0) d.HoWo = 1;
    if (d.dil <= 0) d.dil = 1;
    if (d.stat_tiles) *d.stat_tiles = 0;
    if (d.dmode == DMODE_NCHW_UP2X4 && (d.M & 3)) return IVLN_E_INVALID;
    if (d.Ctot <= 0) d.Ctot = d.dmode == DMODE_NCHW_UP2X4 ? d.M / 4 : d.M;
    if (d.in_img_stride <= 0) d.in_img_stride = (int64_t)d.Cin * d.Hin * d.Win;
    if (d.grp_imgs > 0) {
        if (d.amode != AMODE_MK || d.dmode != DMODE_NCHW || d.N % ((int64_t)d.grp_imgs * d.HoWo) != 0) return IVLN_E_INVALID;
        if (d.a_grp_stride <= 0) d.a_grp_stride = (int64_t)d.M * d.lda;
    }
    if (d.img_run_flags) {
        if (d.dmode != DMODE_NCHW || d.defer_epilogue || d.N % d.HoWo != 0 || d.tile_override == 6 || d.tile_override == 8 ||
            d.tile_override == 9)
            return IVLN_E_INVALID;
        d.splits = 1;
        d.A_split = nullptr;
        if (d.tile_override == 0) d.tile_override = ivln_gemm_vec_eligible(d) ? 7 : 1;
    }
    if (d.residual_after_relu) {
        if (!d.A_split || !d.residual || d.defer_epilogue || d.dmode != DMODE_NCHW || d.fuse_A_split || d.accumulate) return IVLN_E_UNSUPPORTED;
        const int rc = ivln_conv_bf3_launch(d, s, true);
        if (rc != IVLN_OK) return rc;
        if (d.splits_used) *d.splits_used = 1;
        return hipGetLastError() == hipSuccess ? IVLN_OK : IVLN_E_HIP;
    }
    if (d.fuse_A_split) {
        if (!d.A_split || d.defer_epilogue || d.dmode != DMODE_NCHW) return IVLN_E_UNSUPPORTED;
        const int rc = ivln_conv_bf3_launch(d, s, true);
        if (rc != IVLN_OK) return rc;
        if (d.splits_used) *d.splits_used = 1;
        return hipGetLastError() == hipSuccess ? IVLN_OK : IVLN_E_HIP;
    }
    if ((d.tile_override == 0 || d.tile_override >= 9) && d.A_split) {
        const int splits_asked = d.splits;
        float* const stats_asked = d.stat_partials;
        const int rc = ivln_conv_bf3_launch(d, s, d.tile_override >= 9);
        if (rc == IVLN_OK) {
            if (d.splits_used) *d.splits_used = d.splits;
            if (d.splits > 1) launch_splitk_epilogue(d, s);
            return hipGetLastError() == hipSuccess ? IVLN_OK : IVLN_E_HIP;
        }
        d.splits = splits_asked;
        d.stat_partials = stats_asked;
        if (rc != IVLN_E_UNSUPPORTED || d.tile_override >= 9) return rc;
    } else if ((d.tile_override == 0 || d.tile_override == 9) && d.bmode == BMODE_IM2COL_T) {
        const int splits_asked = d.splits;
        const int rc = ivln_wgrad_bf3_launch(d, s, d.tile_override == 9);
        if (rc == IVLN_OK) {
            if (d.splits_used) *d.splits_used = d.splits;
            launch_splitk_epilogue(d, s);
            return hipGetLastError() == hipSuccess ? IVLN_OK : IVLN_E_HIP;
        }
        d.splits = splits_asked;
        if (rc != IVLN_E_UNSUPPORTED || d.tile_override == 9) return rc;
    } else if (d.tile_override >= 9) {
        return IVLN_E_UNSUPPORTED;
    }
    if (d.tile_override == 0 || d.tile_override == 6) {
        int rc = ivln_conv_direct_launch(d, s);
        if (rc == IVLN_E_UNSUPPORTED) rc = ivln_wgrad_direct_launch(d, s);
        if (rc == IVLN_OK) {
            if (d.splits_used) *d.splits_used = d.splits;
            if (d.splits > 1 && !d.defer_epilogue) {
                launch_splitk_epilogue(d, s);
            }
            return hipGetLastError() == hipSuccess ? IVLN_OK : IVLN_E_HIP;
        }
        if (rc != IVLN_E_UNSUPPORTED || d.tile_override == 6) return rc;
    }
    if ((d.tile_override == 0 || d.tile_override == 8) && d.splits <= 1) {
        const int rc = ivln_conv1x1_stream_launch(d, s, d.tile_override == 8);
        if (rc == IVLN_OK) {
            if (d.splits_used) *d.splits_used = 1;
            return hipGetLastError() == hipSuccess ? IVLN_OK : IVLN_E_HIP;
        }
        if (rc != IVLN_E_UNSUPPORTED || d.tile_override == 8) return rc;
    }
    int tile = 0;
    if (d.M <= 32) tile = 1;
    else if (d.N <= 32) tile = 2;
    else {
        auto nblocks = [&](int bm, int bn) { return (int64_t)((d.M + bm - 1) / bm) * ((d.N + bn - 1) / bn); };
        if (nblocks(64, 128) >= 512) tile = 4;
    }
    if (d.tile_override > 0 && d.tile_override <= 5) tile = d.tile_override - 1;
    constexpr int vec_tile_env = -1;
    const bool vec = (d.tile_override == 0 || d.tile_override == 7) && ivln_gemm_vec_eligible(d);
    if (d.tile_override == 7 && !vec) return IVLN_E_UNSUPPORTED;
    const int bk = vec ? 32 : BK;
    if (vec && tile != 1 && tile != 2) tile = vec_tile_env >= 0 ? vec_tile_env : 0;
    if (d.grp_imgs > 0) {
        const int64_t gp = (int64_t)d.grp_imgs * d.HoWo;
        const int bn = tile == 1 ? 128 : (tile == 2 ? 32 : (tile == 3 || tile == 4 ? 128 : 64));
        if (gp % bn != 0) {
            if (gp % 64 == 0) tile = 0;
            else if (gp % 32 == 0) tile = 2;
            else return IVLN_E_UNSUPPORTED;
        }
    }
    const int BM = tile == 1 ? 32 : (tile == 2 || tile == 3 ? 128 : 64);
    const int BN = tile == 1 ? 128 : (tile == 2 ? 32 : (tile == 3 || tile == 4 ? 128 : 64));
    int64_t blocks = (int64_t)((d.M + BM - 1) / BM) * ((d.N + BN - 1) / BN);
    int nk = (d.K + bk - 1) / bk;
    int splits = 1;
    if (d.defer_epilogue && (!d.ws || d.ws_floats < (int64_t)d.M * d.N)) return IVLN_E_INVALID;
    if (d.splits == 0) {
        const int min_tiles = d.defer_epilogue ? 2 : 4;
        constexpr int want_env = 0;
        constexpr int want_nd_env = 0;
        const int64_t want = want_env > 0 ? want_env
                             : (d.defer_epilogue ? 256 : (want_nd_env > 0 ? want_nd_env : 512));
        constexpr int below_env = 0;
        const int64_t below = (below_env > 0 && !d.defer_epilogue) ? below_env : 256;
        if (d.ws && blocks < below && nk >= 2 * min_tiles) {
            splits = (int)((want + blocks - 1) / blocks);
            if (splits > nk / min_tiles) splits = nk / min_tiles;
            constexpr int deep_env = 64;
            const int max_splits = d.defer_epilogue ? (blocks <= 8 ? 64 : (blocks <= 32 ? 32 : 16))
                                                    : (nk >= 4096 ? 256 : (nk >= 512 ? deep_env : 16));
            if (splits > max_splits) splits = max_splits;
            int64_t cap = d.ws_floats / ((int64_t)d.M * d.N);
            if (splits > cap) splits = (int)cap;
            if (splits < 1) splits = 1;
        }
    } else {
        splits = d.splits;
        if (splits > 1 && (!d.ws || d.ws_floats < (int64_t)splits * d.M * d.N)) return IVLN_E_INVALID;
    }
    int tps = (nk + splits - 1) / splits;
    splits = (nk + tps - 1) / tps;
    d.splits = splits;
    int rc;
    if (vec) rc = ivln_gemm_vec_launch(d, s, tile);
    else switch (tile) {
        case 1: rc = launch_tile<1, 4, 1, 1>(d, s); break;
        case 2: rc = launch_tile<4, 1, 1, 1>(d, s); break;
        case 3: rc = launch_tile<2, 2, 2, 2>(d, s); break;
        case 4: rc = launch_tile<2, 2, 1, 2>(d, s); break;
        default: rc = launch_tile<2, 2, 1, 1>(d, s); break;
    }
    if (rc != IVLN_OK) return rc;
    if (d.splits_used) *d.splits_used = splits;
    if (splits > 1 && !d.defer_epilogue) {
        launch_splitk_epilogue(d, s);
    }
    return hipGetLastError() == hipSuccess ? IVLN_OK : IVLN_E_HIP;
}
```

### ivln-ce_amd/csrc/nn_ops.hip

```cpp
#include <hip/hip_runtime.h>
#include <stdint.h>
#include <math.h>
#include "../../include/ivln_hip.h"
#include "gru_seq.h"

namespace {

__device__ __forceinline__ float wave_sum(float v) {
#pragma unroll
    for (int o = 32; o > 0; o >>= 1) v += __shfl_xor(v, o);
    return v;
}
__device__ __forceinline__ float wave_max(float v) {
#pragma unroll
    for (int o = 32; o > 0; o >>= 1) v = fmaxf(v, __shfl_xor(v, o));
    return v;
}
__device__ __forceinline__ float block_sum(float v, float* red) {
    v = wave_sum(v);
    int w = threadIdx.x >> 6, nw = (blockDim.x + 63) >> 6;
    __syncthreads();
    if ((threadIdx.x & 63) == 0) red[w] = v;
    __syncthreads();
    float s = 0.f;
// ... 1558 lines not shown

int ivln_attn_fwd_f32(const float* q, int64_t ldq, const float* k, int64_t k_img_stride, const float* v,
                      int64_t v_img_stride, const int* valid_len, float scale, int rows, int Ck, int Cv, int I,
                      float* out, int64_t ldo, float* save_attn, float* logits_ws, void* stream) {
    return ivln_attn_fwd_idx_f32(q, ldq, k, k_img_stride, v, v_img_stride, valid_len, scale, rows, Ck, Cv, I, out, ldo,
                                 save_attn, logits_ws, nullptr, stream);
}

int ivln_attn_small2_f32(const float* q, int64_t ldq, float scale, int rows, int I, const float* k0,
                         int64_t k0_img_stride, const float* v0, int64_t v0_img_stride, int Ck0, int Cv0, float* out0,
                         int64_t ldo0, const float* k1, int64_t k1_img_stride, const float* v1, int64_t v1_img_stride,
                         int Ck1, int Cv1, float* out1, int64_t ldo1, void* stream) {
    if (I > 32 || I <= 0 || Ck0 > 1024 || Ck1 > 1024 || rows <= 0) return IVLN_E_UNSUPPORTED;
    AttnSet a{k0, v0, out0, k0_img_stride, v0_img_stride, ldo0, Ck0, Cv0};
    AttnSet b{k1, v1, out1, k1_img_stride, v1_img_stride, ldo1, Ck1, Cv1};
    const int sets = k1 ? 2 : 1;
    const int cv = sets == 2 && Cv1 > Cv0 ? Cv1 : Cv0;
    hipLaunchKernelGGL(k_attn_small, dim3(rows, (cv + 15) / 16, sets), dim3(256), 0, (hipStream_t)stream, q, ldq, scale,
                       I, a, b);
    return LAUNCH_OK();
}

int ivln_prev_action_embed_f32(const int64_t* prev_actions, const uint8_t* mask, const float* table, int rows, int E,
                               int n_emb, float* out1, int64_t ld1, float* out2, int64_t ld2, void* stream) {
    hipLaunchKernelGGL(k_prev_action_embed, dim3((rows * E + 255) / 256), dim3(256), 0, (hipStream_t)stream,
                       prev_actions, mask, table, rows, E, n_emb, out1, ld1, out2, ld2);
    return LAUNCH_OK();
}

__global__ void k_tour_memory(const float* __restrict__ mem, int64_t ld_mem, const float* __restrict__ h, int64_t ld_h,
                              const uint8_t* __restrict__ mask, int N, int H, float* __restrict__ out1, int64_t ld1,
                              float* __restrict__ out2, int64_t ld2) {
    const int i = blockIdx.x * blockDim.x + threadIdx.x;
    if (i >= N * H) return;
    const int n = i / H, c = i - n * H;
    float v = mem[(int64_t)n * ld_mem + c];
    if (h) v = fmaxf(v, h[(int64_t)n * ld_h + c]);
    v = mask && !mask[n] ? 0.f : v;
    out1[(int64_t)n * ld1 + c] = v;
    if (out2) out2[(int64_t)n * ld2 + c] = v;
}

int ivln_tour_memory_f32(const float* mem, int64_t ld_mem, const float* h, int64_t ld_h, const uint8_t* mask, int N,
                         int H, float* out1, int64_t ld1, float* out2, int64_t ld2, void* stream) {
    if (N <= 0 || H <= 0 || !mem || !out1) return IVLN_E_INVALID;
    hipLaunchKernelGGL(k_tour_memory, dim3((N * H + 255) / 256), dim3(256), 0, (hipStream_t)stream, mem, ld_mem, h, ld_h,
                       mask, N, H, out1, ld1, out2, ld2);
    return LAUNCH_OK();
}

int ivln_argmax_rows(const float* x, int rows, int C, int64_t* out, void* stream) {
    hipLaunchKernelGGL(k_argmax_rows, dim3((rows + 63) / 64), dim3(64), 0, (hipStream_t)stream, x, rows, C, out);
    return LAUNCH_OK();
}

int ivln_linear_argmax_f32(const float* x, int64_t ldx, const float* W, const float* bias, int rows, int K, int O,
                           int64_t* action, float* logits_out, void* stream) {
    if (O > 8 || O <= 0 || (K & 3) || (ldx & 3) || rows <= 0) return IVLN_E_UNSUPPORTED;
    hipLaunchKernelGGL(k_linear_argmax<false>, dim3(1), dim3(256), 0, (hipStream_t)stream, x, ldx, W, bias, rows, K, O,
                       action, logits_out, (const float*)nullptr, (const float*)nullptr, 0.f, (const double*)nullptr);
    return LAUNCH_OK();
}

int ivln_linear_sample_f32(const float* x, int64_t ldx, const float* W, const float* bias, int rows, int K, int O,
                           const float* u_sample, const float* u_beta, float beta, const double* expert,
                           int64_t* action, float* logits_out, void* stream) {
    if (O > 8 || O <= 0 || (K & 3) || (ldx & 3) || rows <= 0) return IVLN_E_UNSUPPORTED;
    if (!u_sample || (u_beta && !expert)) return IVLN_E_INVALID;
    hipLaunchKernelGGL(k_linear_argmax<true>, dim3(1), dim3(256), 0, (hipStream_t)stream, x, ldx, W, bias, rows, K, O,
                       action, logits_out, u_sample, u_beta, beta, expert);
    return LAUNCH_OK();
}

int ivln_rgb_to_nchw_f32(const uint8_t* rgb, int B, int H, int W, float div, float* out, void* stream) {
    if (B <= 0 || div == 0.f) return IVLN_E_INVALID;
    hipLaunchKernelGGL(k_rgb_to_nchw, dim3(nblk((int64_t)B * H * W)), dim3(256), 0, (hipStream_t)stream, rgb, B, H, W,
                       div, out);
    return LAUNCH_OK();
}

int ivln_adaptive_avgpool2d_f32(const float* x, int N, int C, int H, int W, int OH, int OW, float* out,
                                int64_t out_img_stride, void* stream) {
    if (N <= 0 || OH <= 0 || OW <= 0) return IVLN_E_INVALID;
    if (out_img_stride <= 0) out_img_stride = (int64_t)C * OH * OW;
    hipLaunchKernelGGL(k_adaptive_avgpool2d, dim3(nblk((int64_t)N * C * OH * OW)), dim3(256), 0, (hipStream_t)stream, x,
                       N, C, H, W, OH, OW, out, out_img_stride);
    return LAUNCH_OK();
}

int ivln_argmax_channels_u8(const float* x, int N, int C, int HW, uint8_t* out, void* stream) {
    hipLaunchKernelGGL(k_argmax_channels_u8, dim3(nblk((int64_t)N * HW)), dim3(256), 0, (hipStream_t)stream, x, N, C,
                       HW, out);
    return LAUNCH_OK();
}

int ivln_rgb_resize_normalize_f32(const uint8_t* rgb, int B, int Hi, int Wi, int Ho, int Wo, float* out,
                                  void* stream) {
    if (Hi == Ho && Wi == Wo && ((int64_t)Ho * Wo) % 4 == 0 && !((uintptr_t)rgb & 3) && !((uintptr_t)out & 15)) {
        const int64_t quads = (int64_t)B * Ho * Wo / 4;
        hipLaunchKernelGGL(k_rgb_normalize_x4, dim3(nblk(quads)), dim3(256), 0, (hipStream_t)stream, rgb, quads, Ho * Wo, out);
        return LAUNCH_OK();
    }
    hipLaunchKernelGGL(k_rgb_resize_normalize, dim3(nblk((int64_t)B * 3 * Ho * Wo)), dim3(256), 0,
                       (hipStream_t)stream, rgb, B, Hi, Wi, Ho, Wo, out);
    return LAUNCH_OK();
}

int ivln_affine_f32(const float* x, float* y, int64_t n, float sub, float div, void* stream) {
    hipLaunchKernelGGL(k_affine, dim3(nblk(n)), dim3(256), 0, (hipStream_t)stream, x, y, n, sub, div);
    return LAUNCH_OK();
}

int ivln_add_f32(const float* a, const float* b, float* y, int64_t n, int relu, void* stream) {
    hipLaunchKernelGGL(k_add, dim3(nblk(n)), dim3(256), 0, (hipStream_t)stream, a, b, y, n, relu);
    return LAUNCH_OK();
}

int ivln_copy2d_f32(const float* src, int64_t ld_src, float* dst, int64_t ld_dst, int rows, int cols,
                    int broadcast_rows, void* stream) {
    hipLaunchKernelGGL(k_copy2d, dim3(nblk((int64_t)rows * cols)), dim3(256), 0, (hipStream_t)stream, src, ld_src,
                       dst, ld_dst, rows, cols, broadcast_rows);
    return LAUNCH_OK();
}

int ivln_copy_multi(const void* const* srcs, void* const* dsts, const int64_t* bytes, int n, void* stream) {
    if (n < 0 || n > 8) return IVLN_E_INVALID;
    CopyJobs J;
    int blocks = 0, m = 0;
    for (int j = 0; j < n; ++j) {
        if (bytes[j] <= 0) continue;
        if (!srcs[j] || !dsts[j]) return IVLN_E_INVALID;
        J.src[m] = (const uint8_t*)srcs[j];
        J.dst[m] = (uint8_t*)dsts[j];
        J.bytes[m] = bytes[j];
        J.first_block[m] = blocks;
        blocks += (int)((bytes[j] + COPY_CHUNK - 1) / COPY_CHUNK);
        ++m;
    }
    if (m == 0) return IVLN_OK;
    J.first_block[m] = blocks;
    J.n = m;
    hipLaunchKernelGGL(k_copy_multi, dim3(blocks), dim3(256), 0, (hipStream_t)stream, J);
    return LAUNCH_OK();
}

int ivln_rednet_fwd(const ivln_rednet_op* table, int n_ops, const uint8_t* rgb, const float* depth, uint8_t* labels_out,
                    void* stream) {
    if (!table || n_ops <= 0) return IVLN_E_INVALID;
    for (int k = 0; k < n_ops; ++k) {
        const ivln_rednet_op& op = table[k];
        int rc = IVLN_E_INVALID;
        switch (op.kind) {
            case IVLN_OP_GEMM:
                rc = ivln_gemm_f32(&op.gemm, stream);
                break;
            case IVLN_OP_ADD:
                rc = ivln_add_f32((const float*)op.src0, (const float*)op.src1, (float*)op.dst, op.n, op.i[0], stream);
                break;
            case IVLN_OP_POOL:
                rc = ivln_pool2d_f32((const float*)op.src0, (float*)op.dst, op.i[0], op.i[1], op.i[2], op.i[3], op.i[4],
                                     op.i[5], op.i[6], stream);
                break;
            case IVLN_OP_RGB_NORM: {
                const uint8_t* src = op.src0 ? (const uint8_t*)op.src0 : rgb;
                if (src)
                    rc = ivln_rgb_resize_normalize_f32(src, op.i[0], op.i[1], op.i[2], op.i[3], op.i[4], (float*)op.dst,
                                                       stream);
                break;
            }
            case IVLN_OP_AFFINE: {
                const float* src = op.src0 ? (const float*)op.src0 : depth;
                if (src) rc = ivln_affine_f32(src, (float*)op.dst, op.n, op.f[0], op.f[1], stream);
                break;
            }
            case IVLN_OP_ARGMAX_U8: {
                uint8_t* dst = op.dst ? (uint8_t*)op.dst : labels_out;
                if (dst) rc = ivln_argmax_channels_u8((const float*)op.src0, op.i[0], op.i[1], op.i[2], dst, stream);
                break;
            }
            default:
                break;
        }
        if (rc != IVLN_OK) return rc;
    }
    return IVLN_OK;
}

int ivln_add_multi_f32(const float* const* srcs, float* const* dsts, const int64_t* counts, int n, void* stream) {
    if (n < 0 || n > 64) return IVLN_E_INVALID;
    AddJobs J;
    int blocks = 0, m = 0;
    for (int j = 0; j < n; ++j) {
        if (counts[j] <= 0) continue;
        if (!srcs[j] || !dsts[j]) return IVLN_E_INVALID;
        J.src[m] = srcs[j];
        J.dst[m] = dsts[j];
        J.n[m] = counts[j];
        J.first_block[m] = blocks;
        blocks += (int)((counts[j] + ADD_CHUNK - 1) / ADD_CHUNK);
        ++m;
    }
    if (m == 0) return IVLN_OK;
    J.first_block[m] = blocks;
    J.count = m;
    hipLaunchKernelGGL(k_add_multi, dim3(blocks), dim3(256), 0, (hipStream_t)stream, J);
    return LAUNCH_OK();
}

}
```

### ivln-ce_amd/ops.py

```python
import ctypes as C
import contextlib
import os
from typing import Optional

import torch

from . import _lib
from ._lib import check, f32, i32, i64, lib, stream_ptr, vp
from ._lib import dptr as _dptr


class GemmDesc(C.Structure):

    _fields_ = [
        ("A", vp), ("B", vp), ("D", vp),
        ("M", i32), ("N", i32), ("K", i32),
        ("amode", i32), ("bmode", i32), ("dmode", i32),
        ("lda", i64), ("ldb", i64),
        ("Cin", i32), ("Hin", i32), ("Win", i32), ("Hout", i32), ("Wout", i32),
        ("stride", i32), ("pad", i32), ("dil", i32),
        ("koff", vp), ("kpos", vp),
        ("HoWo", i32), ("Ctot", i32),
        ("in_img_stride", i64),
        ("sDm", i64), ("sDn", i64),
        ("scale", vp), ("shift", vp), ("residual", vp),
        ("relu", i32), ("accumulate", i32),
        ("splits", i32),
        ("ws", vp), ("ws_floats", i64),
        ("defer_epilogue", i32), ("splits_used", C.POINTER(i32)),
        ("tile_override", i32),
        ("A_packed", vp),
        ("no_xcd_remap", i32),
        ("grp_imgs", i32), ("a_grp_stride", i64), ("a_packed_grp_stride", i64),
        ("no_wide_epilogue", i32),
        ("stat_partials", vp), ("stat_tiles", C.POINTER(i32)),
        ("A_split", vp), ("a_split_grp_stride", i64),
        ("split_ok", i32),
        ("img_run_flags", vp),
        ("fuse_A_split", vp), ("fuse_a_grp_stride", i64), ("fuse_scale", vp), ("fuse_shift", vp), ("fuse_M", i32),
        ("residual_after_relu", i32),
        ("real_taps", i32),
    ]


class RednetOp(C.Structure):
    _fields_ = [("kind", i32), ("i", i32 * 7), ("f", f32 * 2), ("n", i64), ("src0", vp), ("src1", vp), ("dst", vp),
                ("gemm", GemmDesc)]


OP_GEMM, OP_ADD, OP_POOL, OP_RGB_NORM, OP_AFFINE, OP_ARGMAX_U8 = range(6)


class OpRecorder:

    def __init__(self):
        self.ops, self.keep, self.unsupported = [], [], []

    def table(self):
        arr = (RednetOp * len(self.ops))()
        for k, op in enumerate(self.ops):
            C.memmove(C.byref(arr, k * C.sizeof(RednetOp)), C.byref(op), C.sizeof(RednetOp))
        return arr


_REC = None


class recording:
    def __enter__(self):
        global _REC
        if _REC is not None:
            raise _lib.IvlnError("ops.recording() does not nest")
        _REC = OpRecorder()
        return _REC

    def __exit__(self, *exc):
        global _REC
        _REC = None
        return False


def _rec(kind, ints=(), floats=(), n=0, src0=None, src1=None, dst=None, gemm=None):
    op = RednetOp()
    op.kind = kind
    for k, v in enumerate(ints):
        op.i[k] = int(v)
    for k, v in enumerate(floats):
        op.f[k] = float(v)
    op.n, op.src0, op.src1, op.dst = int(n), src0, src1, dst
    if gemm is not None:
        C.memmove(C.byref(op, RednetOp.gemm.offset), C.byref(gemm), C.sizeof(GemmDesc))
        op.gemm.splits_used = None
    _REC.ops.append(op)


A_MK, A_KM, A_NCHW_P = 0, 1, 2
B_CONV, B_CONV1X1, B_KN, B_NK, B_IM2COL_T, B_CONVT, B_CONV_K3, B_CONV_K7, B_CONV_K2 = 0, 1, 2, 3, 4, 5, 6, 7, 8
D_NCHW, D_DENSE, D_NCHW_UP2, D_NCHW_UP2X4 = 0, 1, 2, 3

_sigs_done = False


def _L():
    global _sigs_done
    L = lib()
    if not _sigs_done:
        L.ivln_gemm_f32.argtypes = [C.POINTER(GemmDesc), vp]
        L.ivln_groupnorm_f32.argtypes = [vp, vp, vp, vp, vp, i32, i32, i32, i32, f32, i32, i64, i64, i32, i64, i64, i64,
                                         vp, vp, vp]
        L.ivln_bn_fold_f32.argtypes = [vp, vp, vp, vp, vp, f32, i32, vp, vp, vp]
        L.ivln_bn_train_stats_f32.argtypes = [vp, i32, i32, i32, vp, vp, vp, vp, f32, f32, vp, vp, vp, vp, vp, i64, vp]
        L.ivln_scale_shift_relu_avgpool2_f32.argtypes = [vp, vp, vp, vp, i32, i32, i32, i32, i64, i64, i32, i64, vp]
        L.ivln_pool2d_f32.argtypes = [vp, vp, i32, i32, i32, i32, i32, i32, i32, vp]
        L.ivln_map_features_f32.argtypes = [vp, vp, vp, i32, i32, i32, vp]
        L.ivln_embed_lengths.argtypes = [vp, vp, i32, i32, i32, i32, vp, vp, vp]
        L.ivln_lstm_bidir_fwd_f32.argtypes = [vp] * 7 + [i32, i32, i32, vp, vp, vp, vp]
        L.ivln_linear_skinny_f32.argtypes = [vp, i64, vp, vp, vp, i64, i32, i32, i32, i32, vp]
        L.ivln_gru_step_f32.argtypes = [vp, i64, i32, vp, i64, vp, i64, vp, vp, vp, vp, vp, vp, i64, vp, i64, i32, i32,
                                        vp, vp, vp, vp, vp]
        L.ivln_attn_fwd_f32.argtypes = [vp, i64, vp, i64, vp, i64, vp, f32, i32, i32, i32, i32, vp, i64, vp, vp, vp]
        L.ivln_prev_action_embed_f32.argtypes = [vp, vp, vp, i32, i32, i32, vp, i64, vp, i64, vp]
        L.ivln_argmax_rows.argtypes = [vp, i32, i32, vp, vp]
        L.ivln_argmax_channels_u8.argtypes = [vp, i32, i32, i32, vp, vp]
        L.ivln_rgb_resize_normalize_f32.argtypes = [vp, i32, i32, i32, i32, i32, vp, vp]
        L.ivln_affine_f32.argtypes = [vp, vp, i64, f32, f32, vp]
        L.ivln_add_f32.argtypes = [vp, vp, vp, i64, i32, vp]
        L.ivln_copy2d_f32.argtypes = [vp, i64, vp, i64, i32, i32, i32, vp]
        L.ivln_tour_memory_f32.argtypes = [vp, i64, vp, i64, vp, i32, i32, vp, i64, vp, i64, vp]
        _sigs_done = True
    return L


def dptr(t: torch.Tensor) -> int:
    if _REC is not None:
        _REC.keep.append(t)
    return _dptr(t)


def _p(t: Optional[torch.Tensor]):
    if t is None:
        return None
    if not t.is_cuda:
        raise _lib.IvlnError("HIP hot path needs GPU tensors (no CPU fallback); got " + str(t.device))
    if _REC is not None:
        _REC.keep.append(t)
    return t.data_ptr()


_tables = {}
_ws = {}


def conv_tables(cin, kh, kw, hin, win, dil, device, transposed=False):
    key = (cin, kh, kw, hin, win, dil, str(device), transposed)
    t = _tables.get(key)
    if t is None:
        ci = torch.arange(cin, dtype=torch.int64).view(-1, 1, 1)
        a = torch.arange(kh, dtype=torch.int64).view(1, -1, 1)
        b = torch.arange(kw, dtype=torch.int64).view(1, 1, -1)
        if transposed:
            koff = (ci * hin * win + 0 * a + 0 * b).reshape(-1)
        else:
            koff = (ci * hin * win + a * dil * win + b * dil).reshape(-1)
        kpos = (0 * ci + (a << 16) + b).reshape(-1)
        t = (koff.to(torch.int32).to(device), kpos.to(torch.int32).to(device))
        _tables[key] = t
    return t


def splitk_ws(device, floats=8 << 20, slot=0):
    key = (str(device), stream_ptr(), slot)
    w = _ws.get(key)
    if w is None or w.numel() < floats:
        w = torch.empty(floats, dtype=torch.float32, device=device)
        _ws[key] = w
    return w


TILE_OVERRIDE = 0
LINEAR_BWD_SPLIT = True
NO_XCD_REMAP = False
NO_WIDE_EPILOGUE = False
PACK_WEIGHTS = True


def gemm(desc: GemmDesc):
    if TILE_OVERRIDE:
        desc.tile_override = TILE_OVERRIDE
    if NO_XCD_REMAP:
        desc.no_xcd_remap = 1
    if NO_WIDE_EPILOGUE:
        desc.no_wide_epilogue = 1
    check(_L().ivln_gemm_f32(C.byref(desc), stream_ptr()), "ivln_gemm_f32")
    if _REC is not None:
        _rec(OP_GEMM, gemm=desc)


def gemm_soft(desc: GemmDesc) -> bool:
    rc = _L().ivln_gemm_f32(C.byref(desc), stream_ptr())
    if rc == _lib.IVLN_E_UNSUPPORTED:
        return False
    check(rc, "ivln_gemm_f32")
    if _REC is not None:
        _rec(OP_GEMM, gemm=desc)
    return True


_WORK_STREAMS = {}
EAGER_WORK_STREAM = os.environ.get("IVLN_EAGER_WORK_STREAM", "1") != "0"


@contextlib.contextmanager
def eager_work_stream(device=None):
    if not EAGER_WORK_STREAM or not torch.cuda.is_available():
        yield
        return
    dev = torch.device("cuda", torch.cuda.current_device()) if device is None else torch.device(device)
    if dev.type != "cuda" or torch.cuda.is_current_stream_capturing():
        yield
        return
    work = _WORK_STREAMS.get(dev.index)
    if work is None:
        work = _WORK_STREAMS[dev.index] = torch.cuda.Stream(dev)
    cur = torch.cuda.current_stream(dev)
    if cur == work:
        yield
        return
    work.wait_stream(cur)
    try:
        with torch.cuda.stream(work):
            yield
    finally:
        cur.wait_stream(work)


def _epilogue(d: GemmDesc, scale, shift, residual, relu, accumulate=False):
    d.scale, d.shift, d.residual = _p(scale), _p(shift), _p(residual)
    d.relu, d.accumulate = int(bool(relu)), int(bool(accumulate))


_packed = {}


def packed_conv_weights(w, cache=True, split=False):
    import weakref

    G = w.shape[0] if w.dim() == 5 else 1
    Cout, Cin, KH, KW = w.shape[-4:]
    L = _L()
    L.ivln_conv_packed_floats.restype = i64
    L.ivln_conv_packed_floats.argtypes = [i32, i32, i32]
    L.ivln_conv_pack_weights_f32.argtypes = [vp, i32, i32, i32, vp, vp]
    L.ivln_conv_split_words.restype = i64
    L.ivln_conv_split_words.argtypes = [i32, i32, i32]
    L.ivln_conv_split_weights_f32.argtypes = [vp, i32, i32, i32, vp, vp]
    L.ivln_conv_stem_split_words.restype = i64
    L.ivln_conv_stem_split_words.argtypes = [i32, i32]
    L.ivln_conv_stem_split_weights_f32.argtypes = [vp, i32, i32, vp, vp]
    stem = split == "stem"
    if stem:
        n1 = L.ivln_conv_stem_split_words(Cout, Cin) if (G == 1 and KH == 7 and KW == 7) else 0
    else:
        n1 = L.ivln_conv_split_words(Cout, Cin, KH) if split else L.ivln_conv_packed_floats(Cout, Cin, KH)
    if n1 <= 0:
        return None
    n = n1 * G
    wsz = Cout * Cin * KH * KW
    fn, fn_name = ((L.ivln_conv_split_weights_f32, "ivln_conv_split_weights_f32") if split
                   else (L.ivln_conv_pack_weights_f32, "ivln_conv_pack_weights_f32"))

    def _pack(dst):
        if stem:
            check(L.ivln_conv_stem_split_weights_f32(w.data_ptr(), Cout, Cin, dst.data_ptr(), stream_ptr()), "ivln_conv_stem_split_weights_f32")
            return
        for g in range(G):
            check(fn(w.data_ptr() + 4 * g * wsz, Cout, Cin, KH, dst.data_ptr() + 4 * g * n1, stream_ptr()), fn_name)

    if not cache:
        out = torch.empty(n, dtype=torch.float32, device=w.device)
        _pack(out)
        return out
    key = (w.data_ptr(), tuple(w.shape), split)
    stamp = (w._version, WEIGHT_EPOCH)
    cur = torch.cuda.current_stream()
    hit = _packed.get(key)
    if hit is not None and hit.ref() is w and hit.stamp == stamp:
        if hit.settled or hit.stream == cur.cuda_stream:
            return hit.out
        if not torch.cuda.is_current_stream_capturing():
            cur.wait_event(hit.event)
            return hit.out
    capturing = torch.cuda.is_current_stream_capturing()
    same = hit is not None and hit.ref() is w
    if same and not capturing:
        if hit.stream != cur.cuda_stream:
            cur.wait_event(hit.event)
        out = hit.out
    else:
        out = torch.empty(n, dtype=torch.float32, device=w.device)
    _pack(out)
    if capturing:
        return out
    if len(_packed) > 1024:
        _packed.clear()
    ev = torch.cuda.Event()
    ev.record(cur)
    _packed[key] = _Packed(stamp, out, weakref.ref(w), cur.cuda_stream, ev)
    return out


class _Packed:
    __slots__ = ("stamp", "out", "ref", "stream", "event", "settled")

    def __init__(self, stamp, out, ref, stream, event):
        self.stamp, self.out, self.ref, self.stream, self.event, self.settled = stamp, out, ref, stream, event, False


def settle_packed_weights():
    for e in _packed.values():
        e.settled = True


class Deferred:

    def __init__(self, ws, splits, N, C, H, W):
        self.ws, self.splits, self.N, self.C, self.H, self.W = ws, splits, N, C, H, W


SPLIT_BF16 = os.environ.get("IVLN_SPLIT_BF16", "1") != "0"
SPLIT_BF16_WGRAD = os.environ.get("IVLN_SPLIT_BF16_WGRAD", "1") != "0"
SPLIT_BF16_1X1 = int(os.environ.get("IVLN_SPLIT_BF16_1X1", "-1"))
BF3_1X1_KS = os.environ.get("IVLN_BF3_1X1_KS", "1") != "0"
BF3_CONVT = os.environ.get("IVLN_BF3_CONVT", "1") != "0"
BF3_S2 = os.environ.get("IVLN_BF3_S2", "1") != "0"
BF3_STEM = os.environ.get("IVLN_BF3_STEM", "1") != "0"
S2_GATHER = os.environ.get("IVLN_S2_GATHER", "1") != "0"
SPLIT_BF16_MIN_OUT = 1 << 18
_stat_ws = {}
CONV_STATS = os.environ.get("IVLN_CONV_STATS", "1") != "0"


def conv_stat_ws(device, floats):
    key = (str(device), stream_ptr())
    w = _stat_ws.get(key)
    if w is None or w.numel() < floats:
        w = torch.empty(floats, dtype=torch.float32, device=device)
        _stat_ws[key] = w
    return w


def conv2d(x, w, stride=1, pad=0, dil=1, scale=None, shift=None, residual=None, relu=False, out=None, out_ctot=0,
           in_img_stride=0, splitk=True, defer=False, ws_slot=0, weight_is_temp=False, stats=None, run_flags=None,
           residual_after_relu=False):
    N, Cin, H, W = x.shape
    G = w.shape[0] if w.dim() == 5 else 0
    Cout, _, KH, KW = w.shape[-4:]
    if (S2_GATHER and stride == 2 and KH == 1 and KW == 1 and pad == 0 and SPLIT_BF16 and BF3_1X1_KS and not TILE_OVERRIDE
            and Cin >= 64 and Cin % 16 == 0 and H % 2 == 0 and W % 8 == 0 and in_img_stride == 0 and not defer and x.is_contiguous()
            and N * (H // 2) * (W // 2) * Cout >= SPLIT_BF16_MIN_OUT):
        xs = pool2d(x, 1, 2, 0, "max")
        return conv2d(xs, w, 1, 0, dil, scale, shift, residual, relu, out, out_ctot, 0, splitk, defer, ws_slot, weight_is_temp,
                      stats, run_flags, residual_after_relu)
    Ho = (H + 2 * pad - dil * (KH - 1) - 1) // stride + 1
    Wo = (W + 2 * pad - dil * (KW - 1) - 1) // stride + 1
    if defer:
        out = splitk_ws(x.device, slot=ws_slot)
    elif out is None:
        out = torch.empty((N, Cout, Ho, Wo), dtype=torch.float32, device=x.device)
    d = GemmDesc()
    d.A, d.B, d.D = dptr(w), _p(x), _p(out)
    d.M, d.N, d.K = Cout, N * Ho * Wo, Cin * KH * KW
    d.amode, d.dmode = A_MK, D_NCHW
    d.lda = d.K
    d.Cin, d.Hin, d.Win, d.Hout, d.Wout = Cin, H, W, Ho, Wo
    d.stride, d.pad, d.dil = stride, pad, dil
    d.HoWo, d.Ctot = Ho * Wo, out_ctot
    d.in_img_stride = in_img_stride
    if G:
        if N % G or not w.is_contiguous():
            raise _lib.IvlnError("image-grouped conv: N must be a multiple of the weight sets, weights contiguous")
        d.grp_imgs, d.a_grp_stride = N // G, Cout * Cin * KH * KW
    if KH == 1 and KW == 1 and pad == 0:
        d.bmode = B_CONV1X1
        if stride == 1 and Cin in (128, 256) and N * Ho * Wo >= 4096 and PACK_WEIGHTS and w.is_contiguous() and not defer:
            pk = packed_conv_weights(w, cache=not weight_is_temp)
            if pk is not None:
                d.A_packed = dptr(pk)
                d.a_packed_grp_stride = pk.numel() // max(G, 1)
        big_1x1 = stride == 2 or 2.0 * Cout * Cin * N * Ho * Wo >= 4e9
        deep_1x1 = stride == 1 and Cin >= 64 and Cin % 16 == 0 and (Ho * Wo) % 4 == 0 and (Ho >= 2 or TILE_OVERRIDE >= 9) and BF3_1X1_KS
        want_1x1 = TILE_OVERRIDE >= 9 or SPLIT_BF16_1X1 == 1 or (SPLIT_BF16_1X1 != 0 and (big_1x1 or deep_1x1))
        if (want_1x1 and SPLIT_BF16 and stride in (1, 2) and (Cin >= 128 or deep_1x1) and (Cout >= 64 or deep_1x1 or TILE_OVERRIDE in (11, 12, 13)) and Wo % 4 == 0
                and (Wo >= 8 or deep_1x1 or TILE_OVERRIDE in (11, 12, 13)) and w.is_contiguous()
                and not defer and (N * Ho * Wo * Cout >= SPLIT_BF16_MIN_OUT or TILE_OVERRIDE >= 9 or residual_after_relu)):
            sp = packed_conv_weights(w, cache=not weight_is_temp, split=True)
            if sp is not None:
                d.A_split = dptr(sp)
                d.a_split_grp_stride = sp.numel() // max(G, 1)
    elif KH == KW and KH in (3, 7) and dil == 1:
        d.bmode = B_CONV_K3 if KH == 3 else B_CONV_K7
        if stride in (1, 2) and PACK_WEIGHTS and w.is_contiguous():
            pk = packed_conv_weights(w, cache=not weight_is_temp)
            if pk is not None:
                d.A_packed = dptr(pk)
                d.a_packed_grp_stride = pk.numel() // max(G, 1)
        s2_ok = stride == 2 and KH == 3 and BF3_S2 and H % 2 == 0 and W % 4 == 0 and Cin % 16 == 0
        stem_ok = (BF3_STEM and SPLIT_BF16 and stride == 2 and KH == 7 and pad == 3 and Cin in (1, 3) and not G and H == 2 * Ho
                   and W == 2 * Wo and Wo % 128 == 0 and w.is_contiguous() and not defer and not TILE_OVERRIDE and stats is None
                   and run_flags is None)
        if stem_ok:
            sp = packed_conv_weights(w, cache=not weight_is_temp, split="stem")
            if sp is not None:
                d.A_split = dptr(sp)
        if (not stem_ok and SPLIT_BF16 and (stride == 1 or s2_ok) and pad == KH // 2 and Wo % 4 == 0 and Wo >= 8 and w.is_contiguous() and not defer
                and (N * Ho * Wo * Cout >= SPLIT_BF16_MIN_OUT or TILE_OVERRIDE >= 9)):
            sp = packed_conv_weights(w, cache=not weight_is_temp, split=True)
            if sp is not None:
                d.A_split = dptr(sp)
                d.a_split_grp_stride = sp.numel() // max(G, 1)
    else:
        d.bmode = B_CONV
        koff, kpos = conv_tables(Cin, KH, KW, H, W, dil, x.device)
        d.koff, d.kpos = dptr(koff), dptr(kpos)
    _epilogue(d, scale, shift, residual, relu)
    if run_flags is not None:
        if defer or run_flags.dtype != torch.int32 or run_flags.numel() < N or not run_flags.is_cuda:
            raise _lib.IvlnError("conv2d(run_flags): int32 flags per image on the device, not with defer")
        d.img_run_flags, splitk = dptr(run_flags), False
        d._run_flags = run_flags
    if defer:
        ws = splitk_ws(x.device, slot=ws_slot)
        used = i32(0)
        d.ws, d.ws_floats, d.splits, d.defer_epilogue = dptr(ws), ws.numel(), 0, 1
        d.splits_used = C.pointer(used)
        gemm(d)
        return Deferred(ws, used.value, N, Cout, Ho, Wo)
    if splitk:
        ws = splitk_ws(x.device)
        d.ws, d.ws_floats, d.splits = dptr(ws), ws.numel(), 0
    else:
        d.splits = 1
    if residual_after_relu:
        if residual is None or defer or stats is not None or run_flags is not None or TILE_OVERRIDE:
            return None
        d.residual_after_relu, d.splits = 1, 1
        return out if gemm_soft(d) else None
    if stats is not None:
        tiles_max = (N * Ho * Wo + 31) // 32
        sp = conv_stat_ws(x.device, tiles_max * Cout * 3)
        n_tiles = i32(0)
        d.stat_partials, d.stat_tiles = dptr(sp), C.pointer(n_tiles)
        gemm(d)
        if n_tiles.value > 0:
            stats.append((sp, n_tiles.value))
        return out
    gemm(d)
    return out


_ALL_ROWS = {}


def all_rows_flags(rows, device):
    k = (str(device), int(rows))
    if k not in _ALL_ROWS:
        _ALL_ROWS[k] = torch.ones((int(rows),), dtype=torch.int32, device=device)
    return _ALL_ROWS[k]


BF3_FUSE = os.environ.get("IVLN_BF3_FUSE", "1") != "0"


def conv3x3_then_1x1(x, w2, scale2, shift2, w3, scale3, shift3, residual):
    if not (BF3_FUSE and SPLIT_BF16) or TILE_OVERRIDE:
        return None
    N, Cin, H, W = x.shape
    G = w2.shape[0] if w2.dim() == 5 else 0
    Cmid, Cout = w2.shape[-4], w3.shape[-4]
    if (Cmid not in (64, 128) or w2.shape[-1] != 3 or w3.shape[-1] != 1 or w3.shape[-3] != Cmid or W % 32 or H % 4 or Cin % 16 or Cout % 32
            or (w3.dim() == 5) != bool(G) or not (w2.is_contiguous() and w3.is_contiguous() and x.is_contiguous()) or (G and N % G)):
        return None
    sp2, sp3 = packed_conv_weights(w2, split=True), packed_conv_weights(w3, split=True)
    if sp2 is None or sp3 is None:
        return None
    out = torch.empty((N, Cout, H, W), dtype=torch.float32, device=x.device)
    d = GemmDesc()
    d.A, d.B, d.D = dptr(w2), _p(x), _p(out)
    d.M, d.N, d.K = Cmid, N * H * W, Cin * 9
    d.amode, d.bmode, d.dmode = A_MK, B_CONV_K3, D_NCHW
    d.lda = d.K
    d.Cin, d.Hin, d.Win, d.Hout, d.Wout = Cin, H, W, H, W
    d.stride, d.pad, d.dil = 1, 1, 1
    d.HoWo, d.Ctot = H * W, Cout
    if G:
        d.grp_imgs, d.a_grp_stride = N // G, Cmid * Cin * 9
    d.A_split, d.a_split_grp_stride = dptr(sp2), sp2.numel() // max(G, 1)
    d.fuse_A_split, d.fuse_a_grp_stride, d.fuse_M = dptr(sp3), sp3.numel() // max(G, 1), Cout
    d.fuse_scale, d.fuse_shift = _p(scale3), _p(shift3)
    _epilogue(d, scale2, shift2, residual, True)
    d.splits = 1
    return out if gemm_soft(d) else None


def bn_stats_from_partials(partials, tiles, bn, scale, shift, save_mean=None, save_rstd=None, update_running=True):
    mom = bn.momentum if bn.momentum is not None else 0.1
    L = _L()
    L.ivln_bn_stats_from_partials_f32.argtypes = [vp, i32, i32, vp, vp, vp, vp, f32, f32, vp, vp, vp, vp, vp]
    check(
        L.ivln_bn_stats_from_partials_f32(dptr(partials), tiles, bn.num_features, dptr(bn.weight), dptr(bn.bias),
                                          dptr(bn.running_mean) if update_running else None,
                                          dptr(bn.running_var) if update_running else None, mom, bn.eps, dptr(scale),
                                          dptr(shift), _p(save_mean), _p(save_rstd), stream_ptr()),
        "ivln_bn_stats_from_partials_f32",
    )


def conv_transpose2d(x, w_oihw, stride, pad, out_pad, scale=None, shift=None, residual=None, relu=False, out=None):
    N, Cin, H, W = x.shape
    Cout, _, KH, KW = w_oihw.shape
    Ho = (H - 1) * stride - 2 * pad + KH + out_pad
    Wo = (W - 1) * stride - 2 * pad + KW + out_pad
    if out is None:
        out = torch.empty((N, Cout, Ho, Wo), dtype=torch.float32, device=x.device)
    d = GemmDesc()
    d.A, d.B, d.D = dptr(w_oihw), dptr(x), dptr(out)
    d.M, d.N, d.K = Cout, N * Ho * Wo, Cin * KH * KW
    d.amode, d.bmode, d.dmode = A_MK, B_CONVT, D_NCHW
    d.lda = d.K
    d.Cin, d.Hin, d.Win, d.Hout, d.Wout = Cin, H, W, Ho, Wo
    d.stride, d.pad, d.dil = stride, pad, 1
    d.HoWo = Ho * Wo
    koff, kpos = conv_tables(Cin, KH, KW, H, W, 1, x.device, transposed=True)
    d.koff, d.kpos = dptr(koff), dptr(kpos)
    _epilogue(d, scale, shift, residual, relu)
    ws = splitk_ws(x.device)
    d.ws, d.ws_floats, d.splits = dptr(ws), ws.numel(), 0
    gemm(d)
    return out


def convt_s2_classes(w_t, pad):
    Cin, Cout, KH, KW = w_t.shape
    out = []
    for a in (0, 1):
        khs = [(dh, a + pad - 2 * dh) for dh in range(0, KH) if 0 <= a + pad - 2 * dh < KH]
        neg = [dh for dh in range(-KH, 0) if 0 <= a + pad - 2 * dh < KH]
        for b in (0, 1):
            kws = [(dw, b + pad - 2 * dw) for dw in range(0, KW) if 0 <= b + pad - 2 * dw < KW]
            negw = [dw for dw in range(-KW, 0) if 0 <= b + pad - 2 * dw < KW]
            if neg or negw or not khs or not kws or [d for d, _ in khs] != list(range(len(khs))) or \
                    [d for d, _ in kws] != list(range(len(kws))):
                return None
            sub = w_t[:, :, [k for _, k in khs]][:, :, :, [k for _, k in kws]]
            out.append((a, b, sub.permute(1, 0, 2, 3).contiguous()))
    return out


def convt_s2_stack(classes):
    t = max(max(w.shape[2], w.shape[3]) for _, _, w in classes)
    Cout, Cin = classes[0][2].shape[:2]
    W = torch.zeros((Cout, 4, Cin, t, t), dtype=torch.float32, device=classes[0][2].device)
    for a, b, w in classes:
        W[:, 2 * a + b, :, :w.shape[2], :w.shape[3]] = w
    return W.view(4 * Cout, Cin, t, t).contiguous()


STACK_CONVT = os.environ.get("IVLN_CONVT_STACK", "1") != "0"


def conv_transpose2d_s2(x, classes, scale=None, shift=None, residual=None, relu=False, out=None, stacked=None):
    N, Cin, H, W = x.shape
    Cout = classes[0][2].shape[0]
    if out is None:
        out = torch.empty((N, Cout, 2 * H, 2 * W), dtype=torch.float32, device=x.device)
    ws = splitk_ws(x.device)
    todo = [(0, 0, stacked)] if (stacked is not None and STACK_CONVT) else classes
    for a, b, w in todo:
        ta, tb = w.shape[2], w.shape[3]
        d = GemmDesc()
        d.A, d.B, d.D = dptr(w), dptr(x), dptr(out)
        d.M, d.N, d.K = w.shape[0], N * H * W, Cin * ta * tb
        d.amode, d.dmode = A_MK, (D_NCHW_UP2X4 if w.shape[0] != Cout else D_NCHW_UP2)
        d.lda = d.K
        d.Cin, d.Hin, d.Win, d.Hout, d.Wout = Cin, H, W, H, W
        d.stride, d.pad, d.dil = 1, 0, 1
        d.HoWo = H * W
        d.Ctot = Cout
        d.sDm, d.sDn = a, b
        if ta == 1 and tb == 1:
            d.bmode = B_CONV1X1
            if (w is stacked and SPLIT_BF16 and BF3_CONVT and BF3_1X1_KS and Cin >= 64 and Cin % 16 == 0 and W % 4 == 0 and w.is_contiguous()
                    and (N * H * W * w.shape[0] >= SPLIT_BF16_MIN_OUT or TILE_OVERRIDE >= 9)):
                sp = packed_conv_weights(w, split=True)
                if sp is not None:
                    d.A_split = dptr(sp)
                    d.a_split_grp_stride = sp.numel()
        elif ta == 2 and tb == 2:
            d.bmode = B_CONV_K2
            if PACK_WEIGHTS and w.is_contiguous():
                pk = packed_conv_weights(w)
                if pk is not None:
                    d.A_packed = dptr(pk)
            if (w is stacked and SPLIT_BF16 and BF3_CONVT and Cin % 16 == 0 and W % 4 == 0 and W >= 8 and w.is_contiguous()
                    and (N * H * W * w.shape[0] >= SPLIT_BF16_MIN_OUT or TILE_OVERRIDE >= 9)):
                sp = packed_conv_weights(w, split=True)
                if sp is not None:
                    d.A_split = dptr(sp)
                    d.a_split_grp_stride = sp.numel()
                    d.real_taps = sum(c.shape[2] * c.shape[3] for _, _, c in classes)
        else:
            d.bmode = B_CONV
            koff, kpos = conv_tables(Cin, ta, tb, H, W, 1, x.device)
# ... 1132 lines not shown
```

### ivln-ce_amd/rednet.py

```python
import os

import torch
import torch.nn as nn

from . import ops


GROUP_ENCODERS = True


def _conv3x3(cin, cout, stride=1):
    return nn.Conv2d(cin, cout, kernel_size=3, stride=stride, padding=1, bias=False)


class _Folded:

    def __init__(self):
        self.c = {}

    def bn(self, bn: nn.BatchNorm2d):
        k = id(bn)
        if k not in self.c:
            C = bn.num_features
            scale = torch.empty(C, dtype=torch.float32, device=bn.weight.device)
# ... 86 lines not shown
    out = torch.empty((N, Cout, Ho, Wo), dtype=torch.float32, device=x2.device)
    for g in range(G):
        sl = slice(g * B, (g + 1) * B)
        ops.conv2d(x2[sl], w2[g], stride=stride, pad=pad, scale=s2[g * Cout:(g + 1) * Cout], shift=b2[g * Cout:(g + 1) * Cout],
                   residual=residual[sl] if residual is not None else None, relu=relu, out=out[sl])
    return out


def _bottleneck_pair(blk: Bottleneck, blk_d: Bottleneck, x2, f: _Folded):
    residual = x2
    if blk.downsample is not None:
        w, s, b = f.pair(blk.downsample[0], blk.downsample[1], blk_d.downsample[0], blk_d.downsample[1])
        residual = _conv_pair(x2, w, s, b, stride=blk.stride)
    w, s, b = f.pair(blk.conv1, blk.bn1, blk_d.conv1, blk_d.bn1)
    y = _conv_pair(x2, w, s, b, relu=True)
    w, s, b = f.pair(blk.conv2, blk.bn2, blk_d.conv2, blk_d.bn2)
    w3, s3, b3 = f.pair(blk.conv3, blk.bn3, blk_d.conv3, blk_d.bn3)
    if blk.stride == 1:
        out = ops.conv3x3_then_1x1(y, w, s, b, w3, s3, b3, residual)
        if out is not None:
            return out
    y = _conv_pair(y, w, s, b, stride=blk.stride, pad=1, relu=True)
    return _conv_pair(y, w3, s3, b3, residual=residual, relu=True)


class TransBasicBlock(nn.Module):
    expansion = 1

    def __init__(self, inplanes, planes, stride=1, upsample=None, **kwargs):
        super().__init__()
        self.conv1 = _conv3x3(inplanes, inplanes)
        self.bn1 = nn.BatchNorm2d(inplanes)
        self.relu = nn.ReLU(inplace=True)
        if upsample is not None and stride != 1:
            self.conv2 = nn.ConvTranspose2d(inplanes, planes, kernel_size=3, stride=stride, padding=1,
                                            output_padding=1, bias=False)
        else:
            self.conv2 = _conv3x3(inplanes, planes, stride)
        self.bn2 = nn.BatchNorm2d(planes)
        self.upsample = upsample
        self.stride = stride

    def forward_hip(self, x, f: _Folded):
        residual = x
        if self.upsample is not None:
            s, b = f.bn(self.upsample[1])
            up = self.upsample[0]
            if isinstance(up, nn.ConvTranspose2d):
                residual = _convt(x, up, f, scale=s, shift=b)
            else:
                residual = ops.conv2d(x, up.weight, scale=s, shift=b)
        s, b = f.bn(self.bn1)
        y = ops.conv2d(x, self.conv1.weight, pad=1, scale=s, shift=b, relu=True)
        s, b = f.bn(self.bn2)
        if isinstance(self.conv2, nn.ConvTranspose2d):
            return _convt(y, self.conv2, f, scale=s, shift=b, residual=residual, relu=True)
        return ops.conv2d(y, self.conv2.weight, stride=self.stride, pad=1, scale=s, shift=b, residual=residual,
                          relu=True)


class RedNet(nn.Module):
    def __init__(self, cfg):
        super().__init__()
        num_classes = cfg["n_classes"]
        block, transblock, layers = Bottleneck, TransBasicBlock, [3, 4, 6, 3]
        self.inplanes = 64
        self.conv1 = nn.Conv2d(3, 64, kernel_size=7, stride=2, padding=3, bias=False)
        self.bn1 = nn.BatchNorm2d(64)
        self.relu = nn.ReLU(inplace=True)
        self.maxpool = nn.MaxPool2d(kernel_size=3, stride=2, padding=1)
        self.layer1 = self._make_layer(block, 64, layers[0])
        self.layer2 = self._make_layer(block, 128, layers[1], stride=2)
        self.layer3 = self._make_layer(block, 256, layers[2], stride=2)
        self.layer4 = self._make_layer(block, 512, layers[3], stride=2)
        self.inplanes = 64
        self.conv1_d = nn.Conv2d(1, 64, kernel_size=7, stride=2, padding=3, bias=False)
        self.bn1_d = nn.BatchNorm2d(64)
        self.layer1_d = self._make_layer(block, 64, layers[0])
        self.layer2_d = self._make_layer(block, 128, layers[1], stride=2)
        self.layer3_d = self._make_layer(block, 256, layers[2], stride=2)
        self.layer4_d = self._make_layer(block, 512, layers[3], stride=2)
        self.inplanes = 512
        self.deconv1 = self._make_transpose(transblock, 256, 6, stride=2)
        self.deconv2 = self._make_transpose(transblock, 128, 4, stride=2)
        self.deconv3 = self._make_transpose(transblock, 64, 3, stride=2)
        self.deconv4 = self._make_transpose(transblock, 64, 3, stride=2)
        self.agant0 = self._make_agant_layer(64, 64)
        self.agant1 = self._make_agant_layer(64 * 4, 64)
        self.agant2 = self._make_agant_layer(128 * 4, 128)
        self.agant3 = self._make_agant_layer(256 * 4, 256)
        self.agant4 = self._make_agant_layer(512 * 4, 512)
        self.inplanes = 64
        self.final_conv = self._make_transpose(transblock, 64, 3)
        self.final_deconv_custom = nn.ConvTranspose2d(self.inplanes, num_classes, kernel_size=2, stride=2, padding=0,
                                                      bias=True)
        self.out5_conv_custom = nn.Conv2d(256, num_classes, kernel_size=1, stride=1, bias=True)
        self.out4_conv_custom = nn.Conv2d(128, num_classes, kernel_size=1, stride=1, bias=True)
        self.out3_conv_custom = nn.Conv2d(64, num_classes, kernel_size=1, stride=1, bias=True)
        self.out2_conv_custom = nn.Conv2d(64, num_classes, kernel_size=1, stride=1, bias=True)
        self._folded = _Folded()

    def _make_layer(self, block, planes, blocks, stride=1):
        downsample = None
        if stride != 1 or self.inplanes != planes * block.expansion:
            downsample = nn.Sequential(
                nn.Conv2d(self.inplanes, planes * block.expansion, kernel_size=1, stride=stride, bias=False),
                nn.BatchNorm2d(planes * block.expansion),
            )
        layers = [block(self.inplanes, planes, stride, downsample)]
        self.inplanes = planes * block.expansion
        for _ in range(1, blocks):
            layers.append(block(self.inplanes, planes))
        return nn.Sequential(*layers)

    def _make_transpose(self, block, planes, blocks, stride=1):
        upsample = None
        if stride != 1:
            upsample = nn.Sequential(
                nn.ConvTranspose2d(self.inplanes, planes, kernel_size=2, stride=stride, padding=0, bias=False),
                nn.BatchNorm2d(planes),
            )
        elif self.inplanes != planes:
            upsample = nn.Sequential(
                nn.Conv2d(self.inplanes, planes, kernel_size=1, stride=stride, bias=False), nn.BatchNorm2d(planes)
            )
        layers = [block(self.inplanes, self.inplanes) for _ in range(1, blocks)]
        layers.append(block(self.inplanes, planes, stride, upsample))
        self.inplanes = planes
        return nn.Sequential(*layers)

    def _make_agant_layer(self, inplanes, planes):
        return nn.Sequential(
            nn.Conv2d(inplanes, planes, kernel_size=1, stride=1, padding=0, bias=False),
            nn.BatchNorm2d(planes), nn.ReLU(inplace=True),
        )

    def invalidate_folded(self):
        self._folded = _Folded()

    def _seq(self, seq, x):
        for blk in seq:
            x = blk.forward_hip(x, self._folded)
        return x

    def _agant(self, layer, x):
        s, b = self._folded.bn(layer[1])
        return ops.conv2d(x, layer[0].weight, scale=s, shift=b, relu=True)

    def _skip_add(self, up, layer, fuse):
        s, b = self._folded.bn(layer[1])
        out = ops.conv2d(fuse, layer[0].weight, scale=s, shift=b, residual=up, relu=True, residual_after_relu=True) if SKIP_ADD_FUSED else None
        return out if out is not None else ops.add(up, self._agant(layer, fuse))

    def forward(self, rgb, depth):
        assert not self.training, "HIP RedNet is inference-only (the reference freezes it, mapper.py:751-752)"
        f = self._folded
        if GROUP_ENCODERS:
            B = rgb.shape[0]
            S = torch.empty((2 * B, 64, rgb.shape[2] // 2, rgb.shape[3] // 2), dtype=torch.float32, device=rgb.device)
            s, b = f.bn(self.bn1)
            sd, bd = f.bn(self.bn1_d)
            ops.conv2d(depth, self.conv1_d.weight, stride=2, pad=3, scale=sd, shift=bd, relu=True, out=S[B:])
            fuse0 = ops.conv2d(rgb, self.conv1.weight, stride=2, pad=3, scale=s, shift=b, relu=True, out=S[:B], residual=S[B:],
                               residual_after_relu=True) if ops.BF3_STEM else None
            if fuse0 is None:
                ops.conv2d(rgb, self.conv1.weight, stride=2, pad=3, scale=s, shift=b, relu=True, out=S[:B])
                fuse0 = ops.add(S[:B], S[B:], out=S[:B])
            P = ops.pool2d(S, 3, 2, 1, "max")
            fuses = []
            _stage_done("stem")
            for li, (la, lb) in enumerate(((self.layer1, self.layer1_d), (self.layer2, self.layer2_d),
                                           (self.layer3, self.layer3_d), (self.layer4, self.layer4_d))):
                for blk, blk_d in zip(la, lb):
                    P = _bottleneck_pair(blk, blk_d, P, f)
                fuses.append(ops.add(P[:B], P[B:], out=P[:B]))
                _stage_done(f"layer{li + 1}")
            fuse1, fuse2, fuse3, fuse4 = fuses
        else:
            s, b = f.bn(self.bn1)
            x = ops.conv2d(rgb, self.conv1.weight, stride=2, pad=3, scale=s, shift=b, relu=True)
            s, b = f.bn(self.bn1_d)
            d = ops.conv2d(depth, self.conv1_d.weight, stride=2, pad=3, scale=s, shift=b, relu=True)
            fuse0 = ops.add(x, d)
            x = ops.pool2d(fuse0, 3, 2, 1, "max")
            d = ops.pool2d(d, 3, 2, 1, "max")
            x, d = self._seq(self.layer1, x), self._seq(self.layer1_d, d)
            fuse1 = ops.add(x, d)
            x, d = self._seq(self.layer2, fuse1), self._seq(self.layer2_d, d)
            fuse2 = ops.add(x, d)
            x, d = self._seq(self.layer3, fuse2), self._seq(self.layer3_d, d)
            fuse3 = ops.add(x, d)
            x, d = self._seq(self.layer4, fuse3), self._seq(self.layer4_d, d)
            fuse4 = ops.add(x, d)
        x = self._agant(self.agant4, fuse4)
        for di, (seq, ag, fuse) in enumerate(((self.deconv1, self.agant3, fuse3), (self.deconv2, self.agant2, fuse2),
                                              (self.deconv3, self.agant1, fuse1), (self.deconv4, self.agant0, fuse0))):
            x = self._skip_add(self._seq(seq, x), ag, fuse)
            _stage_done(f"deconv{di + 1}")
        x = self._seq(self.final_conv, x)
        fd = self.final_deconv_custom
        return _convt(x, fd, f, shift=fd.bias)


class PredictSemantics:

    CFG = {
        "arch": "rednet", "resnet_pretrained": False, "finetune": True, "SUNRGBD_pretrained_weights": "",
        "n_classes": 13, "upsample_prediction": True, "load_model": "data/rednet_mp3d_best_model.pkl",
    }

    def __init__(self, device, model: RedNet = None, load_weights: bool = True):
        self.device = device
        self.model = model
        self.load_weights = load_weights

    def setup(self):
        if self.model is None:
            self.model = RedNet(self.CFG)
            path = self.CFG["load_model"]
            if self.load_weights and os.path.exists(path):
                state = torch.load(path, map_location="cpu")["model_state"]
                if next(iter(state)).split(".")[0] == "module":
                    state = {".".join(k.split(".")[1:]): v for k, v in state.items()}
                self.model.load_state_dict(state)
            self.model = self.model.to(self.device).eval()
            for p in self.model.parameters():
                p.requires_grad = False

    @torch.no_grad()
    def scores(self, observations):
        if observations.get("rgb", None) is None:
            raise Exception("RGB Sensor not in use")
        self.setup()
        depth = observations["depth"].to(torch.float32).contiguous()
        B, H, W, _ = depth.shape
        rgb = ops.rgb_resize_normalize(observations["rgb"].to(torch.uint8).contiguous(), H, W)
        dn = ops.affine(depth.view(B, 1, H, W), 0.213, 0.285)
        return self.model(rgb, dn)

    USE_PLAN = os.environ.get("IVLN_REDNET_PLAN", "1") != "0"

    def _plan_key(self, rgb, depth):
        return (tuple(rgb.shape), tuple(depth.shape), str(depth.device), ops.stream_ptr(),
                ops.WEIGHT_EPOCH, ops.TILE_OVERRIDE)

    def __call__(self, observations):
        if not self.USE_PLAN or torch.cuda.is_current_stream_capturing():
            return ops.argmax_channels_u8(self.scores(observations))
        if observations.get("rgb", None) is None:
            raise Exception("RGB Sensor not in use")
        self.setup()
        depth = observations["depth"].to(torch.float32).contiguous()
        rgb = observations["rgb"].to(torch.uint8).contiguous()
        B, H, W, _ = depth.shape
        labels = torch.empty((B, 1, H, W), dtype=torch.uint8, device=depth.device)
        plans = self.__dict__.setdefault("_plans", {})
        key = self._plan_key(rgb, depth)
        plan = plans.get(key)
        if plan is None:
            with ops.recording() as rec, torch.no_grad():
                first = ops.argmax_channels_u8(self.scores({"rgb": rgb, "depth": depth}))
            if len(plans) > 8:
                plans.clear()
            plans[key] = (rec.table(), len(rec.ops), rec.keep)
            return first
        ops.rednet_fwd(plan[0], plan[1], rgb, depth, labels)
        return labels
```

Baseline: 2384.

## Fuse argmax labels into final convT epilogue and add strided-read stride-2 1x1 conv

```diff
diff --git a/include/ivln_hip.h b/include/ivln_hip.h
--- a/include/ivln_hip.h
+++ b/include/ivln_hip.h
@@ -66,7 +66,8 @@
 enum { IVLN_D_NCHW = 0,
        IVLN_D_DENSE = 1,
        IVLN_D_NCHW_UP2 = 2,
-       IVLN_D_NCHW_UP2X4 = 3  };
+       IVLN_D_NCHW_UP2X4 = 3,
+       IVLN_D_LABELS_UP2X4 = 4  };
 
 typedef struct ivln_gemm_desc {
     const float* A;
diff --git a/ivln-ce_amd/csrc/conv_bf3.hip b/ivln-ce_amd/csrc/conv_bf3.hip
--- a/ivln-ce_amd/csrc/conv_bf3.hip
+++ b/ivln-ce_amd/csrc/conv_bf3.hip
@@ -896,9 +896,11 @@
     return launch_bf3_ks_tile<2, 32>(d, s, a, gb, nimg);
 }
 
-template <bool WT>
+template <bool WT, bool S2 = false, bool LAB = false>
 __global__ __launch_bounds__(WT ? 256 : 512, 2) void k_conv1x1_bf3_ks(const ivln_gemm_desc p, const unsigned char* a_split, long long a_grp_bytes) {
-    constexpr int NW = WT ? 4 : 8, TN = 4, DA = 4, BN = 128;
+    static_assert(!LAB || (WT && !S2), "labels: the wave-tile form of a stride-1 conv");
+    constexpr int NW = WT ? 4 : 8, TN = 4, DA = LAB ? 2 : 4, BN = 128;
+    constexpr int XD = S2 ? 1 : 2, XL = S2 ? 16 : 8;
     constexpr int LDT = BN + 4;
     constexpr unsigned OOB = 0x80000000u;
     extern __shared__ __attribute__((aligned(16))) unsigned char smem[];
@@ -906,7 +908,7 @@
     const int wave = __builtin_amdgcn_readfirstlane(t >> 6);
     const int half = lane >> 5, l31 = lane & 31;
     const BlockId bid = xcd_block_id(p.no_xcd_remap);
-    const int n0 = WT ? (bid.y * NW + wave) * BN : bid.y * BN, m0 = bid.x * 32;
+    const int n0 = WT ? (bid.y * NW + wave) * BN : bid.y * BN;
     const int nch = p.Cin / CB;
     const int HW = p.HoWo;
     const int cpw = WT ? nch : (nch + NW - 1) / NW;
@@ -916,14 +918,29 @@
 
     const int nq = n0 + 4 * l31;
     const int qimg = nq / HW, qpp = nq - qimg * HW;
-    const unsigned hw4 = (unsigned)HW * 4u;
-    const unsigned xvo = nq < p.N ? (unsigned)(((int64_t)qimg * p.in_img_stride + qpp + (int64_t)(8 * half) * HW) * 4) : OOB;
+    const int HWin = S2 ? p.Hin * p.Win : HW;
+    const unsigned hw4 = (unsigned)HWin * 4u;
+    const int qin = S2 ? (qpp / p.Wout) * 2 * p.Win + (qpp % p.Wout) * 2 : qpp;
+    const unsigned xvo = nq < p.N ? (unsigned)(((int64_t)qimg * p.in_img_stride + qin + (int64_t)(8 * half) * HWin) * 4) : OOB;
     const __amdgpu_buffer_rsrc_t rB = bf3_rsrc(p.B);
-    auto load_x = [&](int c, v4i (&xb)[8]) {
-        const int so = c * CB * HW * 4;
-#pragma unroll
-        for (int j = 0; j < 8; ++j) xb[j] = __builtin_amdgcn_raw_buffer_load_b128(rB, (int)xvo, so + j * (int)hw4, 0);
+    auto load_x = [&](int c, v4i (&xb)[XL]) {
+        const int so = c * CB * HWin * 4;
+#pragma unroll
+        for (int j = 0; j < 8; ++j) {
+            if constexpr (S2) {
+                xb[2 * j] = __builtin_amdgcn_raw_buffer_load_b128(rB, (int)xvo, so + j * (int)hw4, 0);
+                xb[2 * j + 1] = __builtin_amdgcn_raw_buffer_load_b128(rB, (int)(xvo + 16u), so + j * (int)hw4, 0);
+            } else {
+                xb[j] = __builtin_amdgcn_raw_buffer_load_b128(rB, (int)xvo, so + j * (int)hw4, 0);
+            }
+        }
     };
+    auto x_at = [&](const v4i (&xb)[XL], int j, int e) { return __int_as_float(S2 ? xb[2 * j + (e >> 1)][2 * (e & 1)] : xb[j][e]); };
+    float lbv[LAB ? 16 : 1];
+    int lbi[LAB ? 16 : 1];
+    const int mtiles_walk = LAB ? (p.M + 31) / 32 : 1;
+    for (int mtw = 0; mtw < mtiles_walk; ++mtw) {
+    const int m0 = LAB ? mtw * 32 : bid.x * 32;
     const int mt = min(m0 / 32, (p.M + 31) / 32 - 1);
     const __amdgpu_buffer_rsrc_t rA = bf3_rsrc(a_split + (int64_t)grp * a_grp_bytes + (int64_t)mt * nch * (3 * 1024));
     const int c_last = max(c1 - 1, 0);
@@ -942,11 +959,11 @@
     unsigned long long ts1 = ts0, tc_split = 0, tc_load = 0, tc_mfma = 0;
 #endif
     if (c0 < c1 && (!WT || n0 < p.N)) {
-        v4i xb[2][8], ab[DA][3];
+        v4i xb[XD][XL], ab[DA][3];
 #pragma unroll
         for (int d = 0; d < DA; ++d) load_a(c0 + d, ab[d]);
         load_x(c0, xb[0]);
-        load_x(min(c0 + 1, c_last), xb[1]);
+        if constexpr (!S2) load_x(min(c0 + 1, c_last), xb[XD - 1]);
 #ifdef BF3_TIMING
         __builtin_amdgcn_s_waitcnt(0);
         ts1 = lane == 0 ? wall_clock64() : 0ull;
@@ -955,6 +972,7 @@
 #pragma unroll
             for (int k = 0; k < DA; ++k) {
                 const int c = cc + k;
+                const int xi = S2 ? 0 : (k & 1);
                 v4i bq[TN][3];
                 bf16x8 a[3];
 #ifdef BF3_TIMING
@@ -967,9 +985,9 @@
                         for (int i = 0; i < 4; ++i) {
                             uint32_t H, M, L;
 #ifdef BF3_PROBE_NO_SPLIT
-                            H = xb[k & 1][2 * i][e], M = xb[k & 1][2 * i + 1][e], L = H ^ M;
+                            H = __float_as_uint(x_at(xb[xi], 2 * i, e)), M = __float_as_uint(x_at(xb[xi], 2 * i + 1, e)), L = H ^ M;
 #else
-                            split3_pair(__int_as_float(xb[k & 1][2 * i][e]), __int_as_float(xb[k & 1][2 * i + 1][e]), H, M, L);
+                            split3_pair(x_at(xb[xi], 2 * i, e), x_at(xb[xi], 2 * i + 1, e), H, M, L);
 #endif
                             bq[e][0][i] = (int)H, bq[e][1][i] = (int)M, bq[e][2][i] = (int)L;
                         }
@@ -981,7 +999,7 @@
                 const unsigned long long tl1 = __builtin_readcyclecounter();
                 __builtin_amdgcn_sched_barrier(0);
 #endif
-                load_x(min(c + 2, c_last), xb[k & 1]);
+                load_x(min(c + XD, c_last), xb[xi]);
                 load_a(c + DA, ab[k]);
                 __builtin_amdgcn_sched_barrier(0);
 #ifdef BF3_TIMING
@@ -1015,6 +1033,51 @@
 #ifdef BF3_TIMING
     const unsigned long long ts2 = lane == 0 ? wall_clock64() : 0ull;
 #endif
+    if constexpr (LAB) {
+        const float pinf = __builtin_huge_valf();
+        if (mtw == 0) {
+#pragma unroll
+            for (int q = 0; q < 16; ++q) lbv[q] = -pinf, lbi[q] = 255;
+        }
+#pragma unroll
+        for (int r = 0; r < 16; ++r) {
+            const int co = (m0 >> 2) + half + 2 * (r >> 2);
+            const bool valid = m0 + 4 * half + (r & 3) + 8 * (r >> 2) < p.M;
+            const float sh = valid && p.shift ? p.shift[co] : 0.f;
+#pragma unroll
+            for (int e = 0; e < 4; ++e) {
+                const int q = e * 4 + (r & 3);
+                float v = acc[e][r] + sh;
+                v = v != v ? (co == 0 ? pinf : -pinf) : v;
+                const bool take = valid && (v > lbv[q] || (v == lbv[q] && co < lbi[q]));
+                lbv[q] = take ? v : lbv[q], lbi[q] = take ? co : lbi[q];
+            }
+        }
+        if (mtw == mtiles_walk - 1) {
+#pragma unroll
+            for (int q = 0; q < 16; ++q) {
+                const float ov = __shfl_xor(lbv[q], 32);
+                const int oi = __shfl_xor(lbi[q], 32);
+                const bool take = ov > lbv[q] || (ov == lbv[q] && oi < lbi[q]);
+                lbi[q] = take ? oi : lbi[q];
+            }
+            const int n = n0 + 4 * l31;
+            if (n < p.N) {
+                const int img = n / HW, pp = n - img * HW;
+                const int ho = pp / p.Wout, wo = pp - ho * p.Wout;
+                uint32_t w[2] = {0u, 0u};
+#pragma unroll
+                for (int e = 0; e < 4; ++e)
+#pragma unroll
+                    for (int b = 0; b < 2; ++b) {
+                        const uint32_t lab = (uint32_t)(half ? lbi[e * 4 + 2 + b] : lbi[e * 4 + b]) & 255u;
+                        w[e >> 1] |= lab << (8 * (2 * (e & 1) + b));
+                    }
+                uint8_t* const lp = reinterpret_cast<uint8_t*>(p.D) + (((int64_t)img * (2 * p.Hout) + 2 * ho + half) * (2 * p.Wout) + 2 * wo);
+                *reinterpret_cast<uint2*>(lp) = make_uint2(w[0], w[1]);
+            }
+        }
+    } else {
     const bool up = p.dmode == DMODE_NCHW_UP2X4;
     if (WT && up) {
         const int n = n0 + 4 * l31;
@@ -1180,6 +1243,7 @@
         }
     }
     }
+    }
 #ifdef BF3_TIMING
     if (lane == 0) {
         __builtin_amdgcn_s_waitcnt(0);
@@ -1194,10 +1258,15 @@
         g_bf3_stamp[b * 8 + 6] = tc_mfma;
     }
 #endif
+    }
 }
 
 int bf3_1x1_ks_launch(ivln_gemm_desc& d, hipStream_t s, int mode, int form_pin = -1) {
-    if (d.stride != 1 || d.pad != 0 || d.Cin % CB != 0 || d.Cin < 4 * CB || d.stat_partials || d.splits > 1) return IVLN_E_UNSUPPORTED;
+    const bool s2 = d.stride == 2;
+    if (s2 && (d.Hin != 2 * d.Hout || d.Win != 2 * d.Wout || (d.Wout & 3) || d.dmode != DMODE_NCHW)) return IVLN_E_UNSUPPORTED;
+    const bool lab = d.dmode == DMODE_LABELS_UP2X4;
+    if (lab && (s2 || d.scale || d.residual || d.relu || d.accumulate || d.grp_imgs > 0 || d.Ctot > 255 || d.Ctot * 4 != d.M)) return IVLN_E_UNSUPPORTED;
+    if ((d.stride != 1 && !s2) || d.pad != 0 || d.Cin % CB != 0 || d.Cin < 4 * CB || d.stat_partials || d.splits > 1) return IVLN_E_UNSUPPORTED;
     if ((d.HoWo & 3) || (d.in_img_stride & 3) || ((((uintptr_t)d.B) | ((uintptr_t)d.D) | ((uintptr_t)d.residual)) & 15)) return IVLN_E_UNSUPPORTED;
     const int64_t nimg = d.N / d.HoWo;
     if (nimg * d.in_img_stride * 4 >= (int64_t)1 << 31 || nimg * d.Ctot * d.HoWo * 4 >= (int64_t)1 << 31) return IVLN_E_UNSUPPORTED;
@@ -1210,6 +1279,8 @@
     if (form_env) wt = form_env[0] == 'w';
     if (form_pin >= 0) wt = form_pin == 1;
     if (wt && nch > 64) wt = false;
+    if (lab && !wt) return IVLN_E_UNSUPPORTED;
+    if (s2 && !wt) return IVLN_E_UNSUPPORTED;
     if (wt && d.accumulate) return IVLN_E_UNSUPPORTED;
     const int64_t mtiles = (d.M + 31) / 32;
     const int64_t wgs = wt ? (int64_t)((d.N + 511) / 512) * mtiles : (int64_t)((d.N + 127) / 128) * mtiles;
@@ -1224,17 +1295,21 @@
     const long long gb = (long long)(d.a_split_grp_stride * 4);
     if (wt) {
         constexpr size_t lds = 0;
-        dim3 grid((unsigned)mtiles, (unsigned)((d.N + 511) / 512), 1);
-        IVLN_LAUNCH_FAMILY(k_conv1x1_bf3_ks<true>, grid, dim3(256), lds, s, d, a, gb);
+        dim3 grid(lab ? 1u : (unsigned)mtiles, (unsigned)((d.N + 511) / 512), 1);
+        if (lab) IVLN_LAUNCH_FAMILY((k_conv1x1_bf3_ks<true, false, true>), grid, dim3(256), lds, s, d, a, gb);
+        else if (s2) IVLN_LAUNCH_FAMILY((k_conv1x1_bf3_ks<true, true>), grid, dim3(256), lds, s, d, a, gb);
+        else IVLN_LAUNCH_FAMILY(k_conv1x1_bf3_ks<true>, grid, dim3(256), lds, s, d, a, gb);
     } else {
         constexpr size_t lds = (size_t)8 * 32 * (128 + 4) * 4;
         static bool attr_done = false;
         if (!attr_done) {
             if (hipFuncSetAttribute((const void*)k_conv1x1_bf3_ks<false>, hipFuncAttributeMaxDynamicSharedMemorySize, (int)lds) != hipSuccess) return IVLN_E_HIP;
+            if (hipFuncSetAttribute((const void*)k_conv1x1_bf3_ks<false, true>, hipFuncAttributeMaxDynamicSharedMemorySize, (int)lds) != hipSuccess) return IVLN_E_HIP;
             attr_done = true;
         }
         dim3 grid((unsigned)mtiles, (unsigned)((d.N + 127) / 128), 1);
-        IVLN_LAUNCH_FAMILY(k_conv1x1_bf3_ks<false>, grid, dim3(512), lds, s, d, a, gb);
+        if (s2) IVLN_LAUNCH_FAMILY((k_conv1x1_bf3_ks<false, true>), grid, dim3(512), lds, s, d, a, gb);
+        else IVLN_LAUNCH_FAMILY(k_conv1x1_bf3_ks<false>, grid, dim3(512), lds, s, d, a, gb);
     }
     return IVLN_OK;
 }
@@ -1863,7 +1938,8 @@
         if (rc == IVLN_OK && d.stat_tiles) *d.stat_tiles = 0;
         return rc;
     }
-    const bool up1 = KS == 1 && d.dmode == DMODE_NCHW_UP2X4;
+    const bool lab1 = KS == 1 && d.dmode == DMODE_LABELS_UP2X4;
+    const bool up1 = (KS == 1 && d.dmode == DMODE_NCHW_UP2X4) || lab1;
     if (!up1 && d.dmode != (KS == 2 ? DMODE_NCHW_UP2X4 : DMODE_NCHW)) return IVLN_E_UNSUPPORTED;
     if (up1) {
         static const bool convt_off1 = getenv("IVLN_BF3_CONVT") && getenv("IVLN_BF3_CONVT")[0] == '0';
@@ -1912,16 +1988,18 @@
     const int ov = d.tile_override;
     const bool post = d.residual_after_relu != 0;
     const bool ins1 = ov == 11 || ov == 12 || ov == 13 || post, ins3 = ov == 10 || ov == 14 || ov == 15;
+    const bool s2r = ov == 16;
+    if (s2r && (KS != 1 || d.stride != 2 || d.Hin != 2 * d.Hout || d.Win != 2 * d.Wout)) return IVLN_E_UNSUPPORTED;
     if (KS == 1 && ov < 20 && (ks1_env != 0 || ins1) && d.splits <= 1 && !d.defer_epilogue && d.HoWo == d.Hout * d.Wout &&
-        d.K == d.Cin && d.N % d.HoWo == 0 && d.Hout == d.Hin && d.Wout == d.Win) {
+        d.K == d.Cin && d.N % d.HoWo == 0 && ((d.stride == 1 && d.Hout == d.Hin && d.Wout == d.Win) || s2r)) {
         const int rc = bf3_1x1_ks_launch(d, s, (ks1_env == 1 || ins1) ? 1 : 0, ov == 12 ? 0 : (ov == 13 ? 1 : -1));
-        if (rc != IVLN_E_UNSUPPORTED || ins1) {
+        if (rc != IVLN_E_UNSUPPORTED || ins1 || s2r) {
             if (rc == IVLN_OK) g_bf3_flops += 2.0 * d.M * (double)d.N * d.K, ++g_bf3_launches, ++g_bf3_kind[ov == 13 ? 3 : (ov == 12 ? 2 : (d.Cin / CB <= 16 ? 3 : 2))];
             if (rc == IVLN_OK && d.stat_tiles) *d.stat_tiles = 0;
             return rc;
         }
     }
-    if (ins1 || (ins3 && KS != 3)) return IVLN_E_UNSUPPORTED;
+    if (ins1 || s2r || (ins3 && KS != 3)) return IVLN_E_UNSUPPORTED;
     if (KS == 1) {
         if ((d.stride != 1 && d.stride != 2) || d.pad != 0 || d.Hout != (d.Hin - 1) / d.stride + 1 || d.Wout != (d.Win - 1) / d.stride + 1 || d.M < 64)
             return IVLN_E_UNSUPPORTED;
diff --git a/ivln-ce_amd/csrc/gemm_common.h b/ivln-ce_amd/csrc/gemm_common.h
--- a/ivln-ce_amd/csrc/gemm_common.h
+++ b/ivln-ce_amd/csrc/gemm_common.h
@@ -16,7 +16,7 @@
     return bmode == BMODE_CONV_K7 ? 7 : (bmode == BMODE_CONV_K3 ? 3 : (bmode == BMODE_CONV_K2 ? 2 : 0));
 }
 __host__ __device__ constexpr int conv_direct_ci(int KS) { return KS == 7 ? 2 : (KS == 2 ? 16 : 8); }
-enum { DMODE_NCHW = 0, DMODE_DENSE = 1, DMODE_NCHW_UP2 = 2, DMODE_NCHW_UP2X4 = 3 };
+enum { DMODE_NCHW = 0, DMODE_DENSE = 1, DMODE_NCHW_UP2 = 2, DMODE_NCHW_UP2X4 = 3, DMODE_LABELS_UP2X4 = 4 };
 
 __device__ __forceinline__ bool ivln_tile_skipped(const ivln_gemm_desc& p, int n0, int BN) {
     if (!p.img_run_flags) return false;
diff --git a/ivln-ce_amd/csrc/gemm_conv.hip b/ivln-ce_amd/csrc/gemm_conv.hip
--- a/ivln-ce_amd/csrc/gemm_conv.hip
+++ b/ivln-ce_amd/csrc/gemm_conv.hip
@@ -489,8 +489,9 @@
     if (d.HoWo <= 0) d.HoWo = 1;
     if (d.dil <= 0) d.dil = 1;
     if (d.stat_tiles) *d.stat_tiles = 0;
-    if (d.dmode == DMODE_NCHW_UP2X4 && (d.M & 3)) return IVLN_E_INVALID;
-    if (d.Ctot <= 0) d.Ctot = d.dmode == DMODE_NCHW_UP2X4 ? d.M / 4 : d.M;
+    const bool labels = d.dmode == DMODE_LABELS_UP2X4;
+    if ((d.dmode == DMODE_NCHW_UP2X4 || labels) && (d.M & 3)) return IVLN_E_INVALID;
+    if (d.Ctot <= 0) d.Ctot = (d.dmode == DMODE_NCHW_UP2X4 || labels) ? d.M / 4 : d.M;
     if (d.in_img_stride <= 0) d.in_img_stride = (int64_t)d.Cin * d.Hin * d.Win;
     if (d.grp_imgs > 0) {
         if (d.amode != AMODE_MK || d.dmode != DMODE_NCHW || d.N % ((int64_t)d.grp_imgs * d.HoWo) != 0) return IVLN_E_INVALID;
@@ -503,6 +504,13 @@
         d.splits = 1;
         d.A_split = nullptr;
         if (d.tile_override == 0) d.tile_override = ivln_gemm_vec_eligible(d) ? 7 : 1;
+    }
+    if (labels) {
+        if (!d.A_split || d.bmode != BMODE_CONV1X1 || d.defer_epilogue || d.fuse_A_split || d.img_run_flags || d.residual_after_relu) return IVLN_E_UNSUPPORTED;
+        const int rc = ivln_conv_bf3_launch(d, s, d.tile_override >= 9);
+        if (rc != IVLN_OK) return rc;
+        if (d.splits_used) *d.splits_used = 1;
+        return hipGetLastError() == hipSuccess ? IVLN_OK : IVLN_E_HIP;
     }
     if (d.residual_after_relu) {
         if (!d.A_split || !d.residual || d.defer_epilogue || d.dmode != DMODE_NCHW || d.fuse_A_split || d.accumulate) return IVLN_E_UNSUPPORTED;
diff --git a/ivln-ce_amd/csrc/nn_ops.hip b/ivln-ce_amd/csrc/nn_ops.hip
--- a/ivln-ce_amd/csrc/nn_ops.hip
+++ b/ivln-ce_amd/csrc/nn_ops.hip
@@ -1734,6 +1734,13 @@
         int rc = IVLN_E_INVALID;
         switch (op.kind) {
             case IVLN_OP_GEMM:
+                if (op.gemm.dmode == IVLN_D_LABELS_UP2X4 && !op.gemm.D) {
+                    if (!labels_out) break;
+                    ivln_gemm_desc g = op.gemm;
+                    g.D = reinterpret_cast<float*>(labels_out);
+                    rc = ivln_gemm_f32(&g, stream);
+                    break;
+                }
                 rc = ivln_gemm_f32(&op.gemm, stream);
                 break;
             case IVLN_OP_ADD:
diff --git a/ivln-ce_amd/ops.py b/ivln-ce_amd/ops.py
--- a/ivln-ce_amd/ops.py
+++ b/ivln-ce_amd/ops.py
@@ -96,7 +96,7 @@
 
 A_MK, A_KM, A_NCHW_P = 0, 1, 2
 B_CONV, B_CONV1X1, B_KN, B_NK, B_IM2COL_T, B_CONVT, B_CONV_K3, B_CONV_K7, B_CONV_K2 = 0, 1, 2, 3, 4, 5, 6, 7, 8
-D_NCHW, D_DENSE, D_NCHW_UP2, D_NCHW_UP2X4 = 0, 1, 2, 3
+D_NCHW, D_DENSE, D_NCHW_UP2, D_NCHW_UP2X4, D_LABELS_UP2X4 = 0, 1, 2, 3, 4
 
 _sigs_done = False
 
@@ -182,6 +182,8 @@
 NO_XCD_REMAP = False
 NO_WIDE_EPILOGUE = False
 PACK_WEIGHTS = True
+S2_STRIDED = True
+LABELS_EPILOGUE = True
 
 
 def gemm(desc: GemmDesc):
@@ -358,6 +360,27 @@
     if (S2_GATHER and stride == 2 and KH == 1 and KW == 1 and pad == 0 and SPLIT_BF16 and BF3_1X1_KS and not TILE_OVERRIDE
             and Cin >= 64 and Cin % 16 == 0 and H % 2 == 0 and W % 8 == 0 and in_img_stride == 0 and not defer and x.is_contiguous()
             and N * (H // 2) * (W // 2) * Cout >= SPLIT_BF16_MIN_OUT):
+        if S2_STRIDED and SPLIT_BF16_1X1 != 0 and stats is None and run_flags is None and not residual_after_relu and w.is_contiguous():
+            sp = packed_conv_weights(w, cache=not weight_is_temp, split=True)
+            if sp is not None:
+                o = out if out is not None else torch.empty((N, Cout, H // 2, W // 2), dtype=torch.float32, device=x.device)
+                d = GemmDesc()
+                d.A, d.B, d.D = dptr(w), _p(x), _p(o)
+                d.M, d.N, d.K = Cout, N * (H // 2) * (W // 2), Cin
+                d.amode, d.bmode, d.dmode = A_MK, B_CONV1X1, D_NCHW
+                d.lda = d.K
+                d.Cin, d.Hin, d.Win, d.Hout, d.Wout = Cin, H, W, H // 2, W // 2
+                d.stride, d.pad, d.dil = 2, 0, dil
+                d.HoWo, d.Ctot = (H // 2) * (W // 2), out_ctot
+                if G:
+                    if N % G:
+                        raise _lib.IvlnError("image-grouped conv: N must be a multiple of the weight sets")
+                    d.grp_imgs, d.a_grp_stride = N // G, Cout * Cin
+                d.A_split, d.a_split_grp_stride = dptr(sp), sp.numel() // max(G, 1)
+                _epilogue(d, scale, shift, residual, relu)
+                d.splits, d.tile_override, d.no_xcd_remap = 1, 16, int(NO_XCD_REMAP)
+                if gemm_soft(d):
+                    return o
         xs = pool2d(x, 1, 2, 0, "max")
         return conv2d(xs, w, 1, 0, dil, scale, shift, residual, relu, out, out_ctot, 0, splitk, defer, ws_slot, weight_is_temp,
                       stats, run_flags, residual_after_relu)
@@ -458,6 +481,34 @@
     return out
 
 
+def conv_transpose2d_s2_labels(x, stacked, shift=None):
+    N, Cin, H, W = x.shape
+    if not (LABELS_EPILOGUE and STACK_CONVT and SPLIT_BF16 and BF3_CONVT and BF3_1X1_KS and TILE_OVERRIDE in (0, 13) and stacked.shape[2] == 1
+            and stacked.shape[3] == 1 and Cin >= 64 and Cin % 16 == 0 and W % 4 == 0 and stacked.is_contiguous() and x.is_contiguous()
+            and (N * H * W * stacked.shape[0] >= SPLIT_BF16_MIN_OUT or TILE_OVERRIDE >= 9)):
+        return None
+    sp = packed_conv_weights(stacked, split=True)
+    if sp is None:
+        return None
+    out = torch.empty((N, 1, 2 * H, 2 * W), dtype=torch.uint8, device=x.device)
+    d = GemmDesc()
+    d.A, d.B, d.D = dptr(stacked), dptr(x), dptr(out)
+    d.M, d.N, d.K = stacked.shape[0], N * H * W, Cin
+    d.amode, d.bmode, d.dmode = A_MK, B_CONV1X1, D_LABELS_UP2X4
+    d.lda = d.K
+    d.Cin, d.Hin, d.Win, d.Hout, d.Wout = Cin, H, W, H, W
+    d.stride, d.pad, d.dil = 1, 0, 1
+    d.HoWo, d.Ctot = H * W, stacked.shape[0] // 4
+    d.A_split, d.a_split_grp_stride = dptr(sp), sp.numel()
+    _epilogue(d, None, shift, None, False)
+    d.splits, d.no_xcd_remap, d.tile_override = 1, int(NO_XCD_REMAP), TILE_OVERRIDE
+    if not gemm_soft(d):
+        return None
+    if _REC is not None:
+        _REC.ops[-1].gemm.D = None
+    return out
+
+
 _ALL_ROWS = {}
 
 
diff --git a/ivln-ce_amd/rednet.py b/ivln-ce_amd/rednet.py
--- a/ivln-ce_amd/rednet.py
+++ b/ivln-ce_amd/rednet.py
@@ -262,7 +262,7 @@
         out = ops.conv2d(fuse, layer[0].weight, scale=s, shift=b, residual=up, relu=True, residual_after_relu=True) if SKIP_ADD_FUSED else None
         return out if out is not None else ops.add(up, self._agant(layer, fuse))
 
-    def forward(self, rgb, depth):
+    def forward(self, rgb, depth, labels=False):
         assert not self.training, "HIP RedNet is inference-only (the reference freezes it, mapper.py:751-752)"
         f = self._folded
         if GROUP_ENCODERS:
@@ -309,6 +309,10 @@
             _stage_done(f"deconv{di + 1}")
         x = self._seq(self.final_conv, x)
         fd = self.final_deconv_custom
+        if labels:
+            cls = f.classes(fd)
+            lab = ops.conv_transpose2d_s2_labels(x, cls[1], shift=fd.bias) if cls is not None else None
+            return lab if lab is not None else ops.argmax_channels_u8(_convt(x, fd, f, shift=fd.bias))
         return _convt(x, fd, f, shift=fd.bias)
 
 
@@ -338,7 +342,7 @@
                 p.requires_grad = False
 
     @torch.no_grad()
-    def scores(self, observations):
+    def scores(self, observations, labels=False):
         if observations.get("rgb", None) is None:
             raise Exception("RGB Sensor not in use")
         self.setup()
@@ -346,17 +350,17 @@
         B, H, W, _ = depth.shape
         rgb = ops.rgb_resize_normalize(observations["rgb"].to(torch.uint8).contiguous(), H, W)
         dn = ops.affine(depth.view(B, 1, H, W), 0.213, 0.285)
-        return self.model(rgb, dn)
+        return self.model(rgb, dn, labels=labels)
 
     USE_PLAN = os.environ.get("IVLN_REDNET_PLAN", "1") != "0"
 
     def _plan_key(self, rgb, depth):
         return (tuple(rgb.shape), tuple(depth.shape), str(depth.device), ops.stream_ptr(),
-                ops.WEIGHT_EPOCH, ops.TILE_OVERRIDE)
+                ops.WEIGHT_EPOCH, ops.TILE_OVERRIDE, ops.S2_STRIDED, ops.LABELS_EPILOGUE)
 
     def __call__(self, observations):
         if not self.USE_PLAN or torch.cuda.is_current_stream_capturing():
-            return ops.argmax_channels_u8(self.scores(observations))
+            return self.scores(observations, labels=True)
         if observations.get("rgb", None) is None:
             raise Exception("RGB Sensor not in use")
         self.setup()
@@ -369,7 +373,7 @@
         plan = plans.get(key)
         if plan is None:
             with ops.recording() as rec, torch.no_grad():
-                first = ops.argmax_channels_u8(self.scores({"rgb": rgb, "depth": depth}))
+                first = self.scores({"rgb": rgb, "depth": depth}, labels=True)
             if len(plans) > 8:
                 plans.clear()
             plans[key] = (rec.table(), len(rec.ops), rec.keep)
```

Result: no change. 2393, median of 6 (+0.4%).
